# fmazilu/ASR-using-robust-NN

Hardware: AMD Instinct MI355X
Metric: utterances/sec (train, 1 s@16 kHz) (higher is better)
Workload: dtype f32 accumulate, fp16 two-plane split products in the training GEMMs (22-bit operands); 1 GPU; raw 16 kHz waveform -> on-GPU MFCC -> Lipschitz-constrained MLP train step (Adam+NonNeg, simple_norm_constraint rho=0.1), 1xMI355X; global_batch=1024, per_gpu_batch=1024, clip=1 s @ 16 kHz fp32, resident_pool_clips_per_gpu=65536, parallelism=dp1, hip_graph=False

## Files before the change

asr-using-robust-nn_amd/csrc/core.hip:

```cpp
#include "common.h"
#include <map>
#include <mutex>

namespace lipasr {

static thread_local char g_err[512] = "";

void set_error(const char* fmt, ...) {
  va_list ap;
  va_start(ap, fmt);
  vsnprintf(g_err, sizeof(g_err), fmt, ap);
  va_end(ap);
}

int device_cus() {
  static int cached[16] = {};
  int dev = 0; (void)hipGetDevice(&dev);
  int& c = cached[dev & 15];
  if (!c) { hipDeviceProp_t prop; c = hipGetDeviceProperties(&prop, dev) == hipSuccess ? prop.multiProcessorCount : 256; }
  return c;
}

bool ensure_dyn_lds(const void* fn, size_t bytes) {
  if (bytes <= 48 * 1024) return true;
  struct Limit { size_t granted = 0, refused = SIZE_MAX; };
  static std::mutex mu;
  static std::map<std::pair<const void*, int>, Limit> limits;
  int dev = 0; (void)hipGetDevice(&dev);
  std::lock_guard<std::mutex> lock(mu);
  Limit& l = limits[{fn, dev}];
  if (bytes <= l.granted) return true;
  if (bytes >= l.refused) return false;
  if (hipFuncSetAttribute(fn, hipFuncAttributeMaxDynamicSharedMemorySize, (int)bytes) == hipSuccess) { l.granted = bytes; return true; }
  set_error("hipFuncSetAttribute: %zu bytes of dynamic LDS refused: %s", bytes, hipGetErrorString(hipGetLastError()));
  l.refused = bytes;
  return false;
}

void mfcc_plan_free(MfccPlan* p);
void mlp_plan_free(lipasr_mlp* m);
void dolphin_plan_free(DolphinPlan* p);
void psy_plan_free(PsyPlan* p);

}

using namespace lipasr;

extern "C" {

int lipasr_version(void) { return 740; }

const char* lipasr_last_error(void) { return g_err; }

int lipasr_create(int device, lipasr_handle_t* out) {
  LP_CHECK_ARG(out != nullptr, "lipasr_create: out is null");
  int n = 0;
  LP_HIP(hipGetDeviceCount(&n));
  LP_CHECK_ARG(device >= 0 && device < n, "lipasr_create: device %d out of range (have %d)", device, n);
  hipDeviceProp_t prop;
  LP_HIP(hipGetDeviceProperties(&prop, device));
  if (strncmp(prop.gcnArchName, "gfx950", 6) != 0) {
    set_error("lipasr_create: device %d is %s; this library is built for gfx950 only", device, prop.gcnArchName);
    return LIPASR_EUNSUPPORTED;
  }
  DeviceGuard g(device);
  if (!g.ok) { set_error("lipasr_create: hipSetDevice(%d) failed", device); return LIPASR_EHIP; }
  lipasr_ctx* c = new lipasr_ctx();
  c->device = device;
  c->scratch_floats = kScratchFloats;
  if (hipMalloc(&c->scratch, c->scratch_floats * sizeof(float)) != hipSuccess) {
    delete c;
    set_error("lipasr_create: scratch allocation failed");
    return LIPASR_ENOMEM;
  }
  if (hipMemset(c->scratch, 0, c->scratch_floats * sizeof(float)) != hipSuccess) {
    (void)hipFree(c->scratch);
    delete c;
    set_error("lipasr_create: scratch memset failed");
    return LIPASR_EHIP;
  }
  if (hipMalloc(&c->zeros, 256) != hipSuccess || hipMemset(c->zeros, 0, 256) != hipSuccess) {
    (void)hipGetLastError();
    if (c->zeros) (void)hipFree(c->zeros);
    c->zeros = nullptr;
  }
  *out = c;
  return LIPASR_OK;
}

int lipasr_destroy(lipasr_handle_t h) {
  LP_CHECK_ARG(h != nullptr, "lipasr_destroy: null handle");
  DeviceGuard g(h->device);
  (void)hipDeviceSynchronize();
  for (hipGraphExec_t ge : h->graphs)
    if (ge) (void)hipGraphExecDestroy(ge);
  h->graphs.clear();
  for (hipStream_t st : h->streams)
    if (st) (void)hipStreamDestroy(st);
  h->streams.clear();
  std::vector<lipasr_mlp*> mlps;
  mlps.swap(h->mlps);
  for (lipasr_mlp* m : mlps) mlp_plan_free(m);
  std::vector<MfccPlan*> plans;
  plans.swap(h->mfcc_plans);
  for (MfccPlan* p : plans) mfcc_plan_free(p);
  h->mfcc = nullptr;
  std::vector<DolphinPlan*> dolphins;
  dolphins.swap(h->dolphin_plans);
  for (DolphinPlan* p : dolphins) dolphin_plan_free(p);
  std::vector<PsyPlan*> psys;
  psys.swap(h->psy_plans);
  for (PsyPlan* p : psys) psy_plan_free(p);
  for (hipEvent_t e : h->timers) (void)hipEventDestroy(e);
  h->timers.clear();
  if (h->scratch) (void)hipFree(h->scratch);
  if (h->zeros) (void)hipFree(h->zeros);
  delete h;
  return LIPASR_OK;
}

int lipasr_timer_create(lipasr_handle_t h, int* timer_id) {
  LP_CHECK_ARG(h && timer_id, "lipasr_timer_create: null argument");
  DeviceGuard g(h->device);
  hipEvent_t a, b;
  LP_HIP(hipEventCreate(&a));
  LP_HIP(hipEventCreate(&b));
  *timer_id = (int)(h->timers.size() / 2);
  h->timers.push_back(a);
  h->timers.push_back(b);
  return LIPASR_OK;
}

int lipasr_timer_start(lipasr_handle_t h, int id, lipasr_stream_t stream) {
  LP_CHECK_ARG(h && id >= 0 && (size_t)(2 * id + 1) < h->timers.size(), "lipasr_timer_start: bad timer id %d", id);
  LP_HIP(hipEventRecord(h->timers[2 * id], S(stream)));
  return LIPASR_OK;
}

int lipasr_timer_stop(lipasr_handle_t h, int id, lipasr_stream_t stream) {
  LP_CHECK_ARG(h && id >= 0 && (size_t)(2 * id + 1) < h->timers.size(), "lipasr_timer_stop: bad timer id %d", id);
  LP_HIP(hipEventRecord(h->timers[2 * id + 1], S(stream)));
  return LIPASR_OK;
}

int lipasr_timer_elapsed_ms(lipasr_handle_t h, int id, float* ms_host) {
  LP_CHECK_ARG(h && ms_host && id >= 0 && (size_t)(2 * id + 1) < h->timers.size(),
               "lipasr_timer_elapsed_ms: bad argument");
  LP_HIP(hipEventSynchronize(h->timers[2 * id + 1]));
  LP_HIP(hipEventElapsedTime(ms_host, h->timers[2 * id], h->timers[2 * id + 1]));
  return LIPASR_OK;
}

namespace lipasr {
constexpr long long kFlagHardFactor = 4;
__global__ void flag_signal_kernel(int* flag, int value) {
  if (threadIdx.x == 0) __hip_atomic_store(flag, value, __ATOMIC_RELEASE, __HIP_MEMORY_SCOPE_AGENT);
}
__global__ void flag_wait_kernel(const int* flag, int value, int* err, long long soft_ticks) {
  if (threadIdx.x == 0) {
    const long long t0 = wall_clock64();
    bool reported = false;
    while (__hip_atomic_load(flag, __ATOMIC_ACQUIRE, __HIP_MEMORY_SCOPE_AGENT) < value) {
      __builtin_amdgcn_s_sleep(16);
      const long long dt = wall_clock64() - t0;
      if (!reported && dt > soft_ticks) {
        if (__hip_atomic_load(err, __ATOMIC_RELAXED, __HIP_MEMORY_SCOPE_SYSTEM) >= 2) break;
        __hip_atomic_store(err, 1, __ATOMIC_RELAXED, __HIP_MEMORY_SCOPE_SYSTEM);
        reported = true;
      }
      if (dt > kFlagHardFactor * soft_ticks) { __hip_atomic_store(err, 2, __ATOMIC_RELAXED, __HIP_MEMORY_SCOPE_SYSTEM); break; }
    }
  }
}
}

int lipasr_flag_signal(lipasr_handle_t h, int* flag, int value, lipasr_stream_t stream) {
  LP_CHECK_ARG(h && flag, "lipasr_flag_signal: null argument");
  hipLaunchKernelGGL(lipasr::flag_signal_kernel, dim3(1), dim3(64), 0, S(stream), flag, value);
  LP_LAUNCH_CHECK();
  return LIPASR_OK;
}

int lipasr_flag_wait(lipasr_handle_t h, const int* flag, int value, int timeout_ms, int* err, lipasr_stream_t stream) {
  LP_CHECK_ARG(h && flag && err, "lipasr_flag_wait: null argument");
  LP_CHECK_ARG(timeout_ms >= 1 && timeout_ms <= 150000, "lipasr_flag_wait: timeout %d ms outside [1, 150000]", timeout_ms);
  hipLaunchKernelGGL(lipasr::flag_wait_kernel, dim3(1), dim3(64), 0, S(stream), flag, value, err, (long long)timeout_ms * 100000LL);
  LP_LAUNCH_CHECK();
  return LIPASR_OK;
}

int lipasr_graph_begin(lipasr_handle_t h, lipasr_stream_t stream) {
  LP_CHECK_ARG(h != nullptr, "lipasr_graph_begin: null handle");
  LP_HIP(hipStreamBeginCapture(S(stream), hipStreamCaptureModeThreadLocal));
  return LIPASR_OK;
}

int lipasr_graph_end(lipasr_handle_t h, lipasr_stream_t stream, int* graph_id) {
  LP_CHECK_ARG(h && graph_id, "lipasr_graph_end: null argument");
  hipGraph_t graph = nullptr;
  LP_HIP(hipStreamEndCapture(S(stream), &graph));
  hipGraphExec_t exec = nullptr;
  hipError_t e = hipGraphInstantiate(&exec, graph, nullptr, nullptr, 0);
  (void)hipGraphDestroy(graph);
// ... 51 lines not shown
```

asr-using-robust-nn_amd/csrc/mfcc.hip:

```cpp
#include "mfcc_plan.h"
#include <memory>

namespace lipasr {

using namespace tables;

long g_k1_launches[K1_KERNELS] = {};
long g_k1_vjp_launches[K1V_KERNELS] = {};

void mfcc_plan_free(MfccPlan* p) {
  if (!p) return;
  void* ptrs[] = {p->d_hbandh, p->d_groups, p->d_dft, p->d_mel_wlo, p->d_mel_whi, p->d_mel_pstart, p->d_mel_plen, p->d_hband, p->d_lo, p->d_h, p->d_noff, p->d_hann, p->d_tw, p->d_mel_start, p->d_mel_len, p->d_mel_off,
                  p->d_mel_w, p->d_dct, p->d_y, p->d_db, p->d_fmax, p->d_gmel, p->d_part, p->d_gy, p->d_dct_rows, p->d_bin_run, p->d_rt_taps, p->d_rt_t0,
                  p->d_dft_t, p->d_melt_off, p->d_melt_len, p->d_melt_m, p->d_melt_w};
  for (void* q : ptrs)
    if (q) (void)hipFree(q);
  for (hipEvent_t e : p->prof_events) (void)hipEventDestroy(e);
  bdft_tables_free(&p->bd);
  delete p;
}

__global__ __launch_bounds__(256) void add_noise_kernel(float* __restrict__ y, int n, int mode, float p0, float p1,
                                                         uint64_t seed) {
  __shared__ double red[4];
// ... 71 lines not shown
  const bool mfma = p->d_hband && !(p->stage_mask & SM_VALU_RESAMPLER);
  path.resampler = h2 ? MfccPath::RS_H2
                   : p->identity ? MfccPath::RS_COPY
                   : resample_persist_ok(p, wav, fmt) ? MfccPath::RS_PERSIST_F32
                   : mfma ? MfccPath::RS_MFMA
                   : (p->taps == 128 && p->up <= 448) ? MfccPath::RS_REG128 : MfccPath::RS_GENERIC;
  return path;
}
}

using namespace lipasr;

struct lipasr_mfcc : lipasr::MfccPlan {};

namespace lipasr {

static void plan_unregister(MfccPlan* p) {
  if (!p || !p->ctx) return;
  std::vector<MfccPlan*>& v = p->ctx->mfcc_plans;
  for (size_t i = 0; i < v.size(); ++i)
    if (v[i] == p) { v.erase(v.begin() + i); break; }
  if (p->ctx->mfcc == p) p->ctx->mfcc = nullptr;
}

static int plan_build(lipasr_handle_t h, int sr_in, int n_samp, int batch_max, int n_fft, int hop, MfccPlan** out) {
  LP_CHECK_ARG(h != nullptr && out != nullptr, "lipasr_mfcc_plan: null argument");
  const bool dft = !(n_fft == kNFft && hop == kHop);
  if (dft && !(n_fft >= 32 && n_fft <= 32 * kDftMaxTiles * 2 - 2 && hop >= 1 && hop <= n_fft)) {
    set_error("lipasr_mfcc_plan_ex: n_fft=%d hop=%d; supported: 2048/512 (FFT path) or 32 <= n_fft <= %d with "
              "1 <= hop <= n_fft (DFT-contraction path)", n_fft, hop, 32 * kDftMaxTiles * 2 - 2);
    return LIPASR_EUNSUPPORTED;
  }
  LP_CHECK_ARG(sr_in >= 1000 && sr_in <= 384000, "lipasr_mfcc_plan: sr_in=%d outside [1000, 384000]", sr_in);
  LP_CHECK_ARG(n_samp >= 2 && batch_max >= 1, "lipasr_mfcc_plan: n_samp=%d batch_max=%d", n_samp, batch_max);
  DeviceGuard g(h->device);
  std::unique_ptr<MfccPlan, void (*)(MfccPlan*)> guard(new lipasr_mfcc(), mfcc_plan_free);
  MfccPlan* p = guard.get();
  p->ctx = h;
  p->sr_in = sr_in; p->n_samp = n_samp; p->batch_max = batch_max;
  p->identity = (sr_in == kSr);
  resampled_lengths(n_samp, sr_in, kSr, &p->n_valid, &p->n_y);
  if (p->n_y < 2) { set_error("lipasr_mfcc_plan: clip too short after resampling"); return LIPASR_EINVAL; }
  p->n_fft = n_fft; p->hop = hop; p->dft = dft;
  p->rs_target_wgs = h->rs_target_wgs;
  p->n_frames = 1 + p->n_y / hop;
  if (dft && p->n_y <= n_fft / 2) { set_error("lipasr_mfcc_plan_ex: clip shorter than the reflect padding"); return LIPASR_EINVAL; }
  int rc = LIPASR_OK;
  if (!p->identity) {
    Polyphase pp = build_polyphase(sr_in, kSr);
    if (pp.up > 4096 || pp.taps > 2048) {
      set_error("lipasr_mfcc_plan: ratio %d/%d needs %d phases x %d taps; unsupported", pp.up, pp.down, pp.up, pp.taps);
      return LIPASR_EUNSUPPORTED;
    }
    p->up = pp.up; p->down = pp.down; p->taps = pp.taps; p->left = pp.left;
    if ((rc = upload(&p->d_h, pp.h)) != LIPASR_OK || (rc = upload(&p->d_noff, pp.n_off)) != LIPASR_OK) return rc;
    {
      std::vector<float> hb;
      std::vector<int> lo;
      if (build_band_tables(pp, &hb, &lo)) {
        p->n_ptiles = (int)lo.size();
        if ((rc = upload(&p->d_hband, hb)) != LIPASR_OK || (rc = upload(&p->d_lo, lo)) != LIPASR_OK) return rc;
        bool fits = true;
        for (int r = 0; r < (int)lo.size(); ++r) {
          const int first = lo[r] + 1, band0 = first & ~7;
          fits = fits && (first - band0 + kRsBand <= kRhK) && (band0 + kRhK <= kRhRowHalfs);
        }
        if (fits && (rc = upload(&p->d_hbandh, build_band_h2(hb, lo))) != LIPASR_OK) return rc;
      }
    }
    if (!dft && p->d_hband && pp.up == kFuUp && pp.left == 64 && (pp.down % 32) == 0 && pp.down >= 160 && pp.down <= 320 &&
        (kFuQ - 1) * pp.down + lo_max(pp) + 1 + kRsBand <= kFuQ * pp.down + 160) {
      std::vector<int> groups = build_groups(p->n_y, p->n_frames, pp.up);
      if (!groups.empty()) {
        p->n_groups = (int)groups.size() / 4;
        if ((rc = upload(&p->d_groups, groups)) != LIPASR_OK) return rc;
        p->fused = true;
      }
    }
  }
  MelSparse ms = mel_sparse(n_fft);
  if (dft) {
    p->dft_tiles = (1 + n_fft / 2 + 31) / 32;
    p->dft_krows = ((n_fft / 2 + 1 + 2 * kDftGroup - 1) / (2 * kDftGroup)) * (2 * kDftGroup);
    p->dft_rpc = (p->n_y + 2 * (n_fft / 2) + hop - 1) / hop;
    if ((rc = upload(&p->d_dft, dft_table(n_fft, p->dft_krows, p->dft_tiles))) != LIPASR_OK) return rc;
  }
  MelPairs mp = dft ? MelPairs() : mel_pairs();
  if (dft) { mp.wlo.assign(1, 0.f); mp.whi.assign(1, 0.f); mp.start.assign(1, 0); mp.len.assign(1, 0); }
  if (!mp.ok) {
    set_error("lipasr_mfcc_plan: mel filter bank is not a two-filters-per-bin bank");
    return LIPASR_EUNSUPPORTED;
  }
  if ((rc = upload(&p->d_mel_wlo, mp.wlo)) != LIPASR_OK || (rc = upload(&p->d_mel_whi, mp.whi)) != LIPASR_OK ||
      (rc = upload(&p->d_mel_pstart, mp.start)) != LIPASR_OK || (rc = upload(&p->d_mel_plen, mp.len)) != LIPASR_OK ||
      (rc = upload(&p->d_hann, hann_periodic())) != LIPASR_OK || (rc = upload(&p->d_tw, twiddles())) != LIPASR_OK ||
      (rc = upload(&p->d_mel_start, ms.start)) != LIPASR_OK || (rc = upload(&p->d_mel_len, ms.len)) != LIPASR_OK ||
      (rc = upload(&p->d_mel_off, ms.off)) != LIPASR_OK || (rc = upload(&p->d_mel_w, ms.w)) != LIPASR_OK ||
      (rc = upload(&p->d_dct, dct_fragments())) != LIPASR_OK)
    return rc;
  if (!dft && (rc = bdft_tables_build(&p->bd)) != LIPASR_OK) return rc;
  const size_t ny = (size_t)batch_max * p->n_y, ndb = (size_t)batch_max * p->n_frames * 128,
               nfm = (size_t)batch_max * p->n_frames;
  if (hipMalloc(&p->d_y, ny * sizeof(float)) != hipSuccess || hipMalloc(&p->d_db, ndb * sizeof(float)) != hipSuccess ||
      hipMalloc(&p->d_fmax, nfm * sizeof(float)) != hipSuccess) {
    set_error("lipasr_mfcc_plan: intermediate allocation failed");
    return LIPASR_ENOMEM;
  }
  h->mfcc_plans.push_back(p);
  *out = guard.release();
  return LIPASR_OK;
}

static int plan_check(const char* fn, const MfccPlan* p, int batch, int L) {
  LP_CHECK_ARG(p != nullptr, "%s: null plan", fn);
  LP_CHECK_ARG(batch >= 1 && batch <= p->batch_max, "%s: batch %d outside [1, %d]", fn, batch, p->batch_max);
  LP_CHECK_ARG(L >= 1, "%s: utterance_length=%d", fn, L);
  return LIPASR_OK;
}

enum ProfEvent { EV_RESAMPLE_BEGIN, EV_RESAMPLE_END, EV_STFT_BEGIN, EV_STFT_END, EV_DCT_END, kProfEvents };
static hipEvent_t* prof_slot(MfccPlan* p) { return p->prof_n < p->prof_cap ? &p->prof_events[kProfEvents * (size_t)p->prof_n] : nullptr; }

static int plan_resample(MfccPlan* p, const float* wav, int batch, float* y, hipStream_t st) {
  const MfccPath path = pick_mfcc_path(p, wav, 0, false);
  hipEvent_t* ev = prof_slot(p);
  if (ev) LP_HIP(hipEventRecord(ev[EV_RESAMPLE_BEGIN], st));
  int rc = launch_resample(p, path.resampler, wav, 0, nullptr, batch, y, st);
  if (rc != LIPASR_OK) return rc;
  if (ev) {
    LP_HIP(hipEventRecord(ev[EV_RESAMPLE_END], st));
    p->prof_half = true;
  }
  return LIPASR_OK;
}

static int plan_from_22k(MfccPlan* p, const float* y, int batch, int n_y, int L, const double* am, const double* as, float* out,
                         hipStream_t st) {
  LP_CHECK_ARG(n_y == p->n_y, "lipasr_mfcc_from_22k: n_y=%d but the plan was made for %d", n_y, p->n_y);
  LP_CHECK_ARG((am == nullptr) == (as == nullptr), "lipasr_mfcc_from_22k: give both affine arrays or neither");
  const MfccPath path = pick_mfcc_path(p, nullptr, 0, false);
  hipEvent_t* ev = p->prof_half ? prof_slot(p) : nullptr;
  if (ev) LP_HIP(hipEventRecord(ev[EV_STFT_BEGIN], st));
  int rc = launch_from_22k(p, path.stft, y, nullptr, batch, L, am, as, out, st, ev ? ev[EV_STFT_END] : nullptr);
  if (rc != LIPASR_OK) return rc;
  if (ev) {
    LP_HIP(hipEventRecord(ev[EV_DCT_END], st));
    p->prof_half = false;
    p->prof_n++;
  }
  return LIPASR_OK;
}

static int plan_run(MfccPlan* p, const void* wav, int fmt, const int* n_valid, int batch, int L, const double* am, const double* as,
                    float* out, hipStream_t st) {
  LP_CHECK_ARG(wav && out, "lipasr_mfcc: null argument");
  LP_CHECK_ARG(fmt == 0 || fmt == 1, "lipasr_mfcc: sample format %d (0 = float32, 1 = int16 PCM)", fmt);
  LP_CHECK_ARG((am == nullptr) == (as == nullptr), "lipasr_mfcc: give both affine arrays or neither");
  const MfccPath path = pick_mfcc_path(p, wav, fmt, n_valid != nullptr);
  if (path.rc != LIPASR_OK) return path.rc;
  hipEvent_t* ev = p->prof_half ? nullptr : prof_slot(p);
  int rc;
  if (ev) LP_HIP(hipEventRecord(ev[EV_RESAMPLE_BEGIN], st));
  if (path.fused) {
    if (ev) {
      LP_HIP(hipEventRecord(ev[EV_RESAMPLE_END], st));
      LP_HIP(hipEventRecord(ev[EV_STFT_BEGIN], st));
    }
    if ((rc = launch_fused(p, wav, fmt, n_valid, batch, st)) != LIPASR_OK) return rc;
    if (ev) LP_HIP(hipEventRecord(ev[EV_STFT_END], st));
    if ((rc = launch_dct(p, batch, L, am, as, out, n_valid, st)) != LIPASR_OK) return rc;
  } else {
    if ((rc = launch_resample(p, path.resampler, wav, fmt, n_valid, batch, p->d_y, st)) != LIPASR_OK) return rc;
    if (ev) {
      LP_HIP(hipEventRecord(ev[EV_RESAMPLE_END], st));
      LP_HIP(hipEventRecord(ev[EV_STFT_BEGIN], st));
    }
    if ((rc = launch_from_22k(p, path.stft, p->d_y, n_valid, batch, L, am, as, out, st, ev ? ev[EV_STFT_END] : nullptr)) != LIPASR_OK) return rc;
  }
  if (ev) {
    LP_HIP(hipEventRecord(ev[EV_DCT_END], st));
    p->prof_n++;
  }
  return LIPASR_OK;
}

static int vjp_workspaces(const char* fn, MfccPlan* p, size_t n_part) {
  int rc;
  if (!p->d_dct_rows && (rc = upload(&p->d_dct_rows, dct_matrix())) != LIPASR_OK) return rc;
  const size_t ngm = (size_t)p->batch_max * p->n_frames * kNMels, ngy = (size_t)p->batch_max * p->n_y;
  if ((!p->d_gmel && hipMalloc(&p->d_gmel, ngm * sizeof(float)) != hipSuccess) ||
      (!p->d_part && hipMalloc(&p->d_part, n_part * sizeof(float)) != hipSuccess) ||
      (!p->d_gy && hipMalloc(&p->d_gy, ngy * sizeof(float)) != hipSuccess)) {
    (void)hipGetLastError();
    set_error("%s: intermediate allocation failed", fn);
    return LIPASR_ENOMEM;
  }
  return LIPASR_OK;
}

static int vjp_prepare(const char* fn, MfccPlan* p) {
  if (p->vj_ready) return LIPASR_OK;
  DeviceGuard g(p->ctx->device);
  p->vj_groups = (p->n_frames + kVjFrames - 1) / kVjFrames;
  MelPairs mp = mel_pairs();
  std::vector<int> run(kNBins, 0);
  for (int m = 0; m < kNMels; ++m)
    for (int i = 0; i < mp.len[m]; ++i) run[mp.start[m] + i] = m;
  int rc;
  if (!p->d_bin_run && (rc = upload(&p->d_bin_run, run)) != LIPASR_OK) return rc;
  if ((rc = vjp_workspaces(fn, p, (size_t)p->batch_max * p->vj_groups * kVjSeg)) != LIPASR_OK) return rc;
  p->vj_ready = true;
  return LIPASR_OK;
}

static int resample_vjp_prepare(MfccPlan* p) {
  if (p->identity || p->d_rt_taps) return LIPASR_OK;
  DeviceGuard g(p->ctx->device);
  const Polyphase pp = build_polyphase(p->sr_in, kSr);
  const long up = pp.up, down = pp.down;
  auto split = [&](long t, long* q, int* ph) {
    long qq = t / up;
    if (t - qq * up < 0) --qq;
    *q = qq; *ph = (int)(t - qq * up);
  };
  auto pos = [&](long t) { long q; int ph; split(t, &q, &ph); return down * q + pp.n_off[ph]; };
  std::vector<int> t0(pp.down), cnt(pp.down);
  int nt = 0;
  for (int r = 0; r < pp.down; ++r) {
    const long A = (long)r + pp.left - pp.taps, B = (long)r + pp.left - 1;
    long num = A * up, t = num / down;
    if (num - t * down < 0) --t;
    t -= 2;
    while (pos(t) < A) ++t;
    t0[r] = (int)t;
    int c = 0;
    while (pos(t + c) <= B) ++c;
    cnt[r] = c;
    nt = std::max(nt, c);
  }
  std::vector<float> ht((size_t)nt * pp.down, 0.0f);
  for (int r = 0; r < pp.down; ++r)
    for (int i = 0; i < cnt[r]; ++i) {
      long q; int ph;
      split((long)t0[r] + i, &q, &ph);
      const long k = (long)r - (down * q + pp.n_off[ph]) + pp.left - 1;
      if (k >= 0 && k < pp.taps) ht[(size_t)i * pp.down + r] = pp.h[(size_t)ph * pp.taps + k];
    }
  p->rt_nt = nt;
  p->rt_t0min = *std::min_element(t0.begin(), t0.end());
  p->rt_t0max = *std::max_element(t0.begin(), t0.end());
  int rc;
  if ((rc = upload(&p->d_rt_t0, t0)) != LIPASR_OK || (rc = upload(&p->d_rt_taps, ht)) != LIPASR_OK) return rc;
  return LIPASR_OK;
}

static int plan_resample_vjp(MfccPlan* p, const float* gy, int batch, float* gx, hipStream_t st, const int* nv = nullptr) {
  int rc = resample_vjp_prepare(p);
  if (rc != LIPASR_OK) return rc;
  ResampleVjpArgs a;
  a.n_y = p->n_y; a.n_valid = p->n_valid; a.n_samp = p->n_samp; a.up = p->up; a.down = p->down; a.identity = p->identity;
  a.ht = p->d_rt_taps; a.t0 = p->d_rt_t0; a.nt = p->rt_nt; a.t0min = p->rt_t0min; a.t0max = p->rt_t0max;
  a.nv = nv; a.sr_in = p->sr_in;
  return launch_resample_vjp(a, gy, gx, batch, st);
}

static int vjp_short_prepare(const char* fn, MfccPlan* p) {
  if (p->vj_ready) return LIPASR_OK;
  DeviceGuard g(p->ctx->device);
  int n_wgs, seg, rc;
  if ((rc = short_vjp_geometry(p->n_fft, p->hop, p->dft_rpc, p->dft_tiles, p->batch_max, &n_wgs, &seg)) != LIPASR_OK) return rc;
  const int nb = p->dft_tiles * 32, ld = p->dft_tiles * 64;
  const std::vector<float> T = dft_table(p->n_fft, p->dft_krows, p->dft_tiles);
  std::vector<float> TT((size_t)nb * ld, 0.0f);
  for (int b = 0; b < nb; ++b)
    for (int n = 0; n < std::min(nb, p->dft_krows); ++n) {
      const size_t src = (size_t)n * ld + (b >> 5) * 64 + (b & 31), dst = (size_t)b * ld + (n >> 5) * 64 + (n & 31);
      TT[dst] = T[src];
      TT[dst + 32] = T[src + 32];
    }
  const MelSparse ms = mel_sparse(p->n_fft);
  std::vector<int> off(nb, 0), len(nb, 0), mm;
  std::vector<float> ww;
  for (int b = 0; b < nb; ++b) {
    off[b] = (int)mm.size();
    for (int m = 0; m < kNMels; ++m) {
      const int j = b - ms.start[m];
      if (j >= 0 && j < ms.len[m] && ms.w[ms.off[m] + j] != 0.0f) { mm.push_back(m); ww.push_back(ms.w[ms.off[m] + j]); }
    }
    len[b] = (int)mm.size() - off[b];
  }
  if (mm.empty()) { mm.push_back(0); ww.push_back(0.0f); }
  if ((rc = upload(&p->d_melt_off, off)) != LIPASR_OK || (rc = upload(&p->d_melt_len, len)) != LIPASR_OK ||
      (rc = upload(&p->d_melt_m, mm)) != LIPASR_OK || (rc = upload(&p->d_melt_w, ww)) != LIPASR_OK ||
      (rc = vjp_workspaces(fn, p, (size_t)n_wgs * seg)) != LIPASR_OK || (rc = upload(&p->d_dft_t, TT)) != LIPASR_OK)
    return rc;
  p->vj_ready = true;
  return LIPASR_OK;
}

static int ragged_unsupported(const char* fn, const MfccPlan* p) {
  if (!(resample_h2_ok(p, nullptr, 0) && stft2_ok(p))) {
    set_error("%s: per-clip lengths need a 2048/512 plan at 16 kHz or 8 kHz with rows a multiple of 4 samples; this plan is %d Hz, "
              "n_fft %d, rows of %d", fn, p->sr_in, p->n_fft, p->n_samp);
    return LIPASR_EUNSUPPORTED;
  }
  return LIPASR_OK;
}

static int plan_resample_ragged(MfccPlan* p, const void* wav, int fmt, const int* nv, int batch, float* y, hipStream_t st) {
  LP_CHECK_ARG(wav && nv && y, "lipasr_mfcc_plan_resample_ragged: null argument");
  LP_CHECK_ARG(fmt == 0 || fmt == 1, "lipasr_mfcc_plan_resample_ragged: sample format %d (0 = float32, 1 = int16 PCM)", fmt);
  const MfccPath path = pick_mfcc_path(p, wav, fmt, true);
  if (path.rc != LIPASR_OK) return path.rc;
  if (path.fused) {
    set_error("lipasr_mfcc_plan_resample_ragged: this plan runs the fused resample -> STFT kernel for this input (rows of %d samples, "
              "alignment, or plan key 2): it has no resampled signal to return", p->n_samp);
    return LIPASR_EUNSUPPORTED;
  }
  int rc = launch_resample(p, path.resampler, wav, fmt, nv, batch, y, st);
  if (rc != LIPASR_OK) return rc;
  return launch_clear_tail(p, nv, batch, y, st);
}

static int plan_from_22k_ragged(MfccPlan* p, const float* y, const int* nv, int batch, int L, const double* am, const double* as,
                                float* out, hipStream_t st) {
  LP_CHECK_ARG(y && nv && out, "lipasr_mfcc_plan_from_22k_ragged: null argument");
  LP_CHECK_ARG((am == nullptr) == (as == nullptr), "lipasr_mfcc_plan_from_22k_ragged: give both affine arrays or neither");
  const MfccPath path = pick_mfcc_path(p, nullptr, 0, true);
  if (!stft2_ok(p)) {
    set_error("lipasr_mfcc_plan_from_22k_ragged: per-clip lengths need the 2048/512 kernels (n_fft %d, hop %d, stage mask %d)", p->n_fft,
// ... 29 lines not shown
  LP_CHECK_ARG((c.flags & ~(c.entry == VJ_ONE_LENGTH ? 7 : 1)) == 0, "%s: unknown flag bits %d", fn, c.flags);
  if (c.flags & 6) {
    set_error("%s: int16 input and per-clip lengths have no backward pass (float32 rows of one length only)", fn);
    return LIPASR_EUNSUPPORTED;
  }
  if (c.entry == VJ_SHORT && !p->dft) {
    set_error("%s: the short-window backward pass covers the plans made with n_fft, hop other than 2048, 512; this plan is 2048/512 "
              "(lipasr_mfcc_plan_vjp)", fn);
    return LIPASR_EUNSUPPORTED;
  }
  if (c.entry != VJ_SHORT && p->dft) {
    set_error("%s: the backward pass covers the 2048/512 plans; this plan has n_fft %d, hop %d%s", fn, p->n_fft, p->hop,
              c.entry == VJ_ONE_LENGTH ? " (short-window plans: lipasr_mfcc_plan_vjp_short)" : "");
    return LIPASR_EUNSUPPORTED;
  }
  if (c.entry == VJ_ONE_LENGTH && p->n_y <= kNFft) {
    set_error("%s: the backward pass needs clips longer than the reflect padding (n_y %d <= %d)", fn, p->n_y, kNFft);
    return LIPASR_EUNSUPPORTED;
  }
  if (c.entry == VJ_RAGGED) {
    if (c.fmt == 1 && domain == 1) {
      set_error("%s: int16 PCM rows are rows at the plan's input rate (domain 0); the 22 050 Hz signal is float32", fn);
      return LIPASR_EUNSUPPORTED;
    }
    if ((rc = ragged_unsupported(fn, p)) != LIPASR_OK) return rc;
  }
  const MfccPath path = pick_mfcc_path(p, domain == 0 ? c.sig : nullptr, c.fmt, nv != nullptr);
  if (c.entry != VJ_ONE_LENGTH && path.rc != LIPASR_OK) return path.rc;
  if (c.entry == VJ_RAGGED && domain == 0 && path.fused) {
    set_error("%s: this plan runs the fused resample -> STFT kernel for this input (row alignment, or plan key 2), which leaves no "
              "resampled signal behind for the backward pass", fn);
    return LIPASR_EUNSUPPORTED;
  }
  if ((rc = c.entry == VJ_SHORT ? vjp_short_prepare(fn, p) : vjp_prepare(fn, p)) != LIPASR_OK) return rc;
  const MfccPath::Stft stft = p->dft ? MfccPath::ST_DFT : MfccPath::ST_STOCKHAM4;
  const bool reuse_y = (c.flags & 1) && !(c.entry == VJ_ONE_LENGTH && prefers_fused(p));
  const bool reuse_tile = (c.flags & 1) && path.stft == stft && (domain == 1 || reuse_y);
  const float* y = static_cast<const float*>(c.sig);
  if (domain == 0) {
    if (!reuse_y && (rc = launch_resample(p, path.resampler, c.sig, c.fmt, nv, batch, p->d_y, st)) != LIPASR_OK) return rc;
    y = p->d_y;
  }
  if (!reuse_tile && (rc = launch_from_22k(p, stft, y, nv, batch, L, nullptr, nullptr, nullptr, st, nullptr, true)) != LIPASR_OK) return rc;
  MfccVjpArgs a;
  a.y = y; a.n_y = p->n_y; a.n_frames = p->n_frames; a.batch = batch; a.L = L;
  a.db = p->d_db; a.fmax = p->d_fmax; a.g_feat = c.g_feat; a.aff_scale = c.scale; a.dct_rows = p->d_dct_rows;
  a.hann = p->d_hann; a.tw = reinterpret_cast<const float2*>(p->d_tw);
  a.mel_wlo = p->d_mel_wlo; a.mel_whi = p->d_mel_whi; a.bin_run = p->d_bin_run;
  a.gmel = p->d_gmel; a.part = p->d_part; a.n_groups = p->vj_groups;
  a.gy = domain == 0 ? p->d_gy : c.g_sig;
  if (c.entry == VJ_SHORT) {
    if ((rc = launch_mfcc_vjp_db(a, st)) != LIPASR_OK) return rc;
    ShortVjpArgs s;
    s.y = y; s.table = p->d_dft; s.table_t = p->d_dft_t; s.gmel = p->d_gmel;
    s.melt_off = p->d_melt_off; s.melt_len = p->d_melt_len; s.melt_m = p->d_melt_m; s.melt_w = p->d_melt_w;
    s.n_y = p->n_y; s.batch = batch; s.hop = p->hop; s.n_fft = p->n_fft; s.k_rows = p->dft_krows; s.n_tiles = p->dft_tiles;
    s.rpc = p->dft_rpc; s.n_frames = p->n_frames; s.total_rows = batch * p->dft_rpc; s.seg = 0;
    s.part = p->d_part; s.gy = a.gy;
    rc = launch_short_vjp(s, st);
  } else {
    rc = nv ? launch_mfcc_vjp(a, st, nv, p->sr_in, p->n_samp) : launch_mfcc_vjp(a, st);
  }
  if (rc != LIPASR_OK) return rc;
  if (domain == 0) return plan_resample_vjp(p, p->d_gy, batch, c.g_sig, st, nv);
  return LIPASR_OK;
}

static int plan_profile_begin(MfccPlan* p, int max_calls) {
  LP_CHECK_ARG(p != nullptr && max_calls >= 1 && max_calls <= 100000, "lipasr_mfcc_profile_begin: bad argument");
  DeviceGuard g(p->ctx->device);
  while ((int)p->prof_events.size() < kProfEvents * max_calls) {
    hipEvent_t e;
    LP_HIP(hipEventCreate(&e));
    p->prof_events.push_back(e);
  }
  p->prof_cap = max_calls;
  p->prof_n = 0;
  p->prof_half = false;
  return LIPASR_OK;
}

static int plan_profile_end(MfccPlan* p, float* avg_ms3, int* n_calls) {
  LP_CHECK_ARG(p && avg_ms3 && n_calls, "lipasr_mfcc_profile_end: null argument");
  double acc[3] = {0, 0, 0};
  static const int kFrom[3] = {EV_RESAMPLE_BEGIN, EV_STFT_BEGIN, EV_STFT_END}, kTo[3] = {EV_RESAMPLE_END, EV_STFT_END, EV_DCT_END};
  for (int i = 0; i < p->prof_n; ++i) {
    hipEvent_t* ev = &p->prof_events[kProfEvents * (size_t)i];
    LP_HIP(hipEventSynchronize(ev[EV_DCT_END]));
    for (int k = 0; k < 3; ++k) {
      float ms = 0.0f;
      LP_HIP(hipEventElapsedTime(&ms, ev[kFrom[k]], ev[kTo[k]]));
      acc[k] += ms;
    }
  }
  *n_calls = p->prof_n;
  for (int k = 0; k < 3; ++k) avg_ms3[k] = p->prof_n ? (float)(acc[k] / p->prof_n) : 0.0f;
  p->prof_cap = 0;
  p->prof_n = 0;
  p->prof_half = false;
  return LIPASR_OK;
}

static int plan_set(MfccPlan* p, int key, int value) {
  LP_CHECK_ARG(p != nullptr, "lipasr_mfcc_set: null plan");
  LP_CHECK_ARG(key >= 0 && key <= 4, "lipasr_mfcc_set: unknown key %d", key);
  if (key == 3) LP_CHECK_ARG(value >= 4 && value <= 4096 && (value & 3) == 0, "lipasr_mfcc_set: frames per workgroup %d (a multiple of 4)", value);
  if (key == 1) LP_CHECK_ARG(value >= 1 && value <= 4096, "lipasr_mfcc_set: resampler workgroup target %d", value);
  switch (key) {
    case 0: p->stage_mask = value; break;
    case 1: p->rs_target_wgs = value; break;
    case 2: p->prefer_fused = value != 0; break;
    case 3: p->bd_seg = value; break;
    default: p->bd_fuse_dct = value != 0; break;
  }
  return LIPASR_OK;
}

}

extern "C" {

int lipasr_mfcc_create(lipasr_handle_t h, int sr_in, int n_samp_max, int batch_max, int n_fft, int hop, lipasr_mfcc_t* out) {
  LP_CHECK_ARG(out != nullptr, "lipasr_mfcc_create: out is null");
  MfccPlan* p = nullptr;
  int rc = plan_build(h, sr_in, n_samp_max, batch_max, n_fft, hop, &p);
  if (rc != LIPASR_OK) return rc;
  *out = static_cast<lipasr_mfcc*>(p);
  return LIPASR_OK;
}

int lipasr_mfcc_destroy(lipasr_mfcc_t p) {
  LP_CHECK_ARG(p != nullptr, "lipasr_mfcc_destroy: null plan");
  DeviceGuard g(p->ctx->device);
  plan_unregister(p);
  mfcc_plan_free(p);
  return LIPASR_OK;
}

int lipasr_mfcc_plan_dims(lipasr_mfcc_t p, int* n_y, int* n_frames, int* fused) {
  LP_CHECK_ARG(p && n_y && n_frames, "lipasr_mfcc_plan_dims: null argument");
  *n_y = p->n_y;
  *n_frames = p->n_frames;
  if (fused) *fused = p->fused ? 1 : 0;
  return LIPASR_OK;
}

int lipasr_mfcc_extract(lipasr_mfcc_t p, const void* wav, int sample_format, const int* n_valid, int batch, int utterance_length,
                        const double* affine_mean, const double* affine_scale, float* out, lipasr_stream_t stream) {
  int rc = plan_check("lipasr_mfcc_extract", p, batch, utterance_length);
  if (rc != LIPASR_OK) return rc;
  return plan_run(p, wav, sample_format, n_valid, batch, utterance_length, affine_mean, affine_scale, out, S(stream));
}

int lipasr_mfcc_plan_resample(lipasr_mfcc_t p, const float* wav, int batch, float* y, lipasr_stream_t stream) {
  int rc = plan_check("lipasr_mfcc_plan_resample", p, batch, 1);
  if (rc != LIPASR_OK) return rc;
  LP_CHECK_ARG(wav && y, "lipasr_mfcc_plan_resample: null argument");
  return plan_resample(p, wav, batch, y, S(stream));
}

int lipasr_mfcc_plan_from_22k(lipasr_mfcc_t p, const float* y, int batch, int n_y, int utterance_length, const double* affine_mean,
                              const double* affine_scale, float* out, lipasr_stream_t stream) {
  int rc = plan_check("lipasr_mfcc_plan_from_22k", p, batch, utterance_length);
  if (rc != LIPASR_OK) return rc;
  LP_CHECK_ARG(y && out, "lipasr_mfcc_plan_from_22k: null argument");
  return plan_from_22k(p, y, batch, n_y, utterance_length, affine_mean, affine_scale, out, S(stream));
}

int lipasr_mfcc_plan_vjp(lipasr_mfcc_t p, const float* sig, int domain, int batch, int utterance_length, const double* affine_scale,
                         const float* g_feat, float* g_sig, int flags, lipasr_stream_t stream) {
  return plan_vjp(p, {"lipasr_mfcc_plan_vjp", VJ_ONE_LENGTH, sig, 0, nullptr, domain, batch, utterance_length, affine_scale, g_feat, g_sig, flags},
                  S(stream));
}

int lipasr_mfcc_plan_vjp_short(lipasr_mfcc_t p, const float* sig, int domain, int batch, int utterance_length, const double* affine_scale,
                               const float* g_feat, float* g_sig, int flags, lipasr_stream_t stream) {
  return plan_vjp(p, {"lipasr_mfcc_plan_vjp_short", VJ_SHORT, sig, 0, nullptr, domain, batch, utterance_length, affine_scale, g_feat, g_sig, flags},
                  S(stream));
}

int lipasr_mfcc_plan_vjp_ragged(lipasr_mfcc_t p, const void* sig, int sample_format, const int* n_valid, int domain, int batch,
                                int utterance_length, const double* affine_scale, const float* g_feat, float* g_sig, int flags,
                                lipasr_stream_t stream) {
  return plan_vjp(p, {"lipasr_mfcc_plan_vjp_ragged", VJ_RAGGED, sig, sample_format, n_valid, domain, batch, utterance_length, affine_scale,
                      g_feat, g_sig, flags},
                  S(stream));
}

int lipasr_mfcc_plan_resample_ragged(lipasr_mfcc_t p, const void* wav, int sample_format, const int* n_valid, int batch, float* y,
                                     lipasr_stream_t stream) {
  int rc = plan_check("lipasr_mfcc_plan_resample_ragged", p, batch, 1);
  if (rc != LIPASR_OK) return rc;
  return plan_resample_ragged(p, wav, sample_format, n_valid, batch, y, S(stream));
}

int lipasr_mfcc_plan_from_22k_ragged(lipasr_mfcc_t p, const float* y, const int* n_valid, int batch, int utterance_length,
                                     const double* affine_mean, const double* affine_scale, float* out, lipasr_stream_t stream) {
  int rc = plan_check("lipasr_mfcc_plan_from_22k_ragged", p, batch, utterance_length);
  if (rc != LIPASR_OK) return rc;
  return plan_from_22k_ragged(p, y, n_valid, batch, utterance_length, affine_mean, affine_scale, out, S(stream));
}

int lipasr_mfcc_plan_resample_vjp(lipasr_mfcc_t p, const float* g_y, int batch, float* g_wav, lipasr_stream_t stream) {
  int rc = plan_check("lipasr_mfcc_plan_resample_vjp", p, batch, 1);
  if (rc != LIPASR_OK) return rc;
  LP_CHECK_ARG(g_y && g_wav, "lipasr_mfcc_plan_resample_vjp: null argument");
  return plan_resample_vjp(p, g_y, batch, g_wav, S(stream));
}

int lipasr_mfcc_plan_profile_begin(lipasr_mfcc_t p, int max_calls) { return plan_profile_begin(p, max_calls); }
int lipasr_mfcc_plan_profile_end(lipasr_mfcc_t p, float* avg_ms3, int* n_calls) { return plan_profile_end(p, avg_ms3, n_calls); }
int lipasr_mfcc_plan_set(lipasr_mfcc_t p, int key, int value) { return plan_set(p, key, value); }

long lipasr_debug_k1_launches(int kernel) { return (kernel >= 0 && kernel < K1_KERNELS) ? g_k1_launches[kernel] : -1; }

int lipasr_debug_mfcc_stage(lipasr_mfcc_t p, int which, int batch, float* out, lipasr_stream_t stream) {
  LP_CHECK_ARG(p != nullptr && out != nullptr, "lipasr_debug_mfcc_stage: null argument");
  LP_CHECK_ARG(batch >= 1 && batch <= p->batch_max, "lipasr_debug_mfcc_stage: batch %d outside [1, %d]", batch, p->batch_max);
  LP_CHECK_ARG(which >= 0 && which <= 2, "lipasr_debug_mfcc_stage: unknown stage %d (0 dB tile, 1 frame maxima, 2 resampled signal)", which);
  const float* src = which == 0 ? p->d_db : which == 1 ? p->d_fmax : p->d_y;
  const size_t row = which == 0 ? (size_t)p->n_frames * 128 : which == 1 ? (size_t)p->n_frames : (size_t)p->n_y;
  DeviceGuard g(p->ctx->device);
  LP_HIP(hipMemcpyAsync(out, src, (size_t)batch * row * sizeof(float), hipMemcpyDeviceToDevice, S(stream)));
  return LIPASR_OK;
}

long lipasr_debug_k1_vjp_launches(int kernel) { return (kernel >= 0 && kernel < K1V_KERNELS) ? g_k1_vjp_launches[kernel] : -1; }

int lipasr_debug_mfcc_vjp_stage(lipasr_mfcc_t p, int which, int batch, float* out, lipasr_stream_t stream) {
  LP_CHECK_ARG(p != nullptr && out != nullptr, "lipasr_debug_mfcc_vjp_stage: null argument");
  LP_CHECK_ARG(batch >= 1 && batch <= p->batch_max, "lipasr_debug_mfcc_vjp_stage: batch %d outside [1, %d]", batch, p->batch_max);
  LP_CHECK_ARG(which >= 0 && which <= 1, "lipasr_debug_mfcc_vjp_stage: unknown stage %d (0 Gmel, 1 g_y of a domain-0 call)", which);
  LP_CHECK_ARG(p->vj_ready && p->d_gmel && p->d_gy, "lipasr_debug_mfcc_vjp_stage: the plan has run no backward pass yet (no workspaces)");
  const float* src = which == 0 ? p->d_gmel : p->d_gy;
  const size_t row = which == 0 ? (size_t)p->n_frames * 128 : (size_t)p->n_y;
  DeviceGuard g(p->ctx->device);
  LP_HIP(hipMemcpyAsync(out, src, (size_t)batch * row * sizeof(float), hipMemcpyDeviceToDevice, S(stream)));
  return LIPASR_OK;
}

int lipasr_debug_mfcc_stage_put(lipasr_mfcc_t p, int which, int batch, const float* in, lipasr_stream_t stream) {
  LP_CHECK_ARG(p != nullptr && in != nullptr, "lipasr_debug_mfcc_stage_put: null argument");
  LP_CHECK_ARG(batch >= 1 && batch <= p->batch_max, "lipasr_debug_mfcc_stage_put: batch %d outside [1, %d]", batch, p->batch_max);
  LP_CHECK_ARG(which >= 0 && which <= 1, "lipasr_debug_mfcc_stage_put: unknown stage %d (0 dB tile, 1 frame maxima)", which);
  float* dst = which == 0 ? p->d_db : p->d_fmax;
  const size_t row = which == 0 ? (size_t)p->n_frames * 128 : (size_t)p->n_frames;
  DeviceGuard g(p->ctx->device);
  LP_HIP(hipMemcpyAsync(dst, in, (size_t)batch * row * sizeof(float), hipMemcpyDeviceToDevice, S(stream)));
  return LIPASR_OK;
}

int lipasr_mfcc_plan(lipasr_handle_t h, int sr_in, int n_samp, int batch_max) {
  return lipasr_mfcc_plan_ex(h, sr_in, n_samp, batch_max, kNFft, kHop);
}

int lipasr_mfcc_plan_ex(lipasr_handle_t h, int sr_in, int n_samp, int batch_max, int n_fft, int hop) {
  LP_CHECK_ARG(h != nullptr, "lipasr_mfcc_plan: null handle");
  MfccPlan* p = nullptr;
  int rc = plan_build(h, sr_in, n_samp, batch_max, n_fft, hop, &p);
  if (rc != LIPASR_OK) return rc;
  if (h->mfcc) {
    DeviceGuard g(h->device);
    MfccPlan* old = h->mfcc;
    plan_unregister(old);
    mfcc_plan_free(old);
  }
  h->mfcc = p;
  return LIPASR_OK;
}

int lipasr_mfcc_dims(lipasr_handle_t h, int* n_y, int* n_frames) {
  LP_CHECK_ARG(h && n_y && n_frames, "lipasr_mfcc_dims: null argument");
  if (!h->mfcc) { set_error("lipasr_mfcc_dims: call lipasr_mfcc_plan first"); return LIPASR_ESTATE; }
  *n_y = h->mfcc->n_y;
  *n_frames = h->mfcc->n_frames;
  return LIPASR_OK;
}

static int mfcc_check(const char* fn, lipasr_handle_t h, int batch, int L) {
  LP_CHECK_ARG(h != nullptr, "%s: null handle", fn);
  if (!h->mfcc) { set_error("%s: call lipasr_mfcc_plan first", fn); return LIPASR_ESTATE; }
  return plan_check(fn, h->mfcc, batch, L);
}

int lipasr_resample_f32(lipasr_handle_t h, const float* wav, int batch, float* y, lipasr_stream_t stream) {
  int rc = mfcc_check("lipasr_resample_f32", h, batch, 1);
  if (rc != LIPASR_OK) return rc;
  LP_CHECK_ARG(wav && y, "lipasr_resample_f32: null argument");
  return plan_resample(h->mfcc, wav, batch, y, S(stream));
}

int lipasr_mfcc_from_22k(lipasr_handle_t h, const float* y, int batch, int n_y, int utterance_length,
                         const double* affine_mean, const double* affine_scale, float* out, lipasr_stream_t stream) {
  int rc = mfcc_check("lipasr_mfcc_from_22k", h, batch, utterance_length);
  if (rc != LIPASR_OK) return rc;
  LP_CHECK_ARG(y && out, "lipasr_mfcc_from_22k: null argument");
  return plan_from_22k(h->mfcc, y, batch, n_y, utterance_length, affine_mean, affine_scale, out, S(stream));
}

int lipasr_mfcc_f32(lipasr_handle_t h, const float* wav, int batch, int utterance_length, const double* affine_mean,
                    const double* affine_scale, float* out, lipasr_stream_t stream) {
  int rc = mfcc_check("lipasr_mfcc_f32", h, batch, utterance_length);
  if (rc != LIPASR_OK) return rc;
  LP_CHECK_ARG(wav && out, "lipasr_mfcc_f32: null argument");
  LP_CHECK_ARG((affine_mean == nullptr) == (affine_scale == nullptr), "lipasr_mfcc_f32: give both affine arrays or neither");
  return plan_run(h->mfcc, wav, 0, nullptr, batch, utterance_length, affine_mean, affine_scale, out, S(stream));
}

int lipasr_mfcc_i16(lipasr_handle_t h, const int16_t* pcm, const int* n_valid, int batch, int utterance_length,
                    const double* affine_mean, const double* affine_scale, float* out, lipasr_stream_t stream) {
  int rc = mfcc_check("lipasr_mfcc_i16", h, batch, utterance_length);
  if (rc != LIPASR_OK) return rc;
  return plan_run(h->mfcc, pcm, 1, n_valid, batch, utterance_length, affine_mean, affine_scale, out, S(stream));
}

int lipasr_mfcc_profile_begin(lipasr_handle_t h, int max_calls) {
  LP_CHECK_ARG(h != nullptr, "lipasr_mfcc_profile_begin: bad argument");
  if (!h->mfcc) { set_error("lipasr_mfcc_profile_begin: call lipasr_mfcc_plan first"); return LIPASR_ESTATE; }
  return plan_profile_begin(h->mfcc, max_calls);
}

int lipasr_mfcc_profile_end(lipasr_handle_t h, float* avg_ms3, int* n_calls) {
  LP_CHECK_ARG(h && avg_ms3 && n_calls, "lipasr_mfcc_profile_end: null argument");
  if (!h->mfcc) { set_error("lipasr_mfcc_profile_end: call lipasr_mfcc_plan first"); return LIPASR_ESTATE; }
  return plan_profile_end(h->mfcc, avg_ms3, n_calls);
}

int lipasr_add_noise_f32(lipasr_handle_t h, float* y, int batch, int n, int mode, float p0, float p1, uint64_t seed,
                         lipasr_stream_t stream) {
  LP_CHECK_ARG(h && y, "lipasr_add_noise_f32: null argument");
  LP_CHECK_ARG(batch >= 1 && n >= 1, "lipasr_add_noise_f32: bad shape %dx%d", batch, n);
  LP_CHECK_ARG(mode >= 0 && mode <= 2, "lipasr_add_noise_f32: mode %d", mode);
  hipLaunchKernelGGL(add_noise_kernel, dim3(batch), dim3(256), 0, S(stream), y, n, mode, p0, p1, seed);
  LP_LAUNCH_CHECK();
  return LIPASR_OK;
}

int lipasr_debug_set(lipasr_handle_t h, int key, int value) {
  LP_CHECK_ARG(h != nullptr, "lipasr_debug_set: null handle");
  LP_CHECK_ARG(key >= 0 && key <= 2, "lipasr_debug_set: unknown key %d", key);
  if (!h->mfcc) { set_error("lipasr_debug_set: call lipasr_mfcc_plan first"); return LIPASR_ESTATE; }
  int rc = plan_set(h->mfcc, key, value);
  if (rc == LIPASR_OK && key == 1) h->rs_target_wgs = value;
  return rc;
}

int lipasr_debug_table(int which, int sr_in, float* out, int cap) {
  std::vector<float> v;
  switch (which) {
    case 0: v = hann_periodic(); break;
    case 1: v = dct_matrix(); break;
    case 2: v = mel_dense(); break;
    case 3: case 4: case 5: case 6: case 7: {
      LP_CHECK_ARG(sr_in >= 1000 && sr_in != kSr, "lipasr_debug_table: sr_in=%d", sr_in);
      Polyphase pp = build_polyphase(sr_in, kSr);
      if (which == 3) v = pp.h;
      else if (which == 4) v = {(float)pp.up, (float)pp.down, (float)pp.taps, (float)pp.left};
      else if (which == 5) v.assign(pp.n_off.begin(), pp.n_off.end());
      else {
        std::vector<float> hb;
        std::vector<int> lo;
        if (!build_band_tables(pp, &hb, &lo)) { set_error("lipasr_debug_table: no banded form for sr_in=%d", sr_in); return LIPASR_EUNSUPPORTED; }
        if (which == 6) v = hb;
        else v.assign(lo.begin(), lo.end());
      }
      break;
    }
    case 8: {
      MelPairs mp = mel_pairs();
      LP_CHECK_ARG(mp.ok, "lipasr_debug_table: mel bank has no pair form");
      v.assign((size_t)kNMels * kNBins, 0.0f);
      for (int m = 0; m < kNMels; ++m)
        for (int i = 0; i < mp.len[m]; ++i) {
          const int b = mp.start[m] + i;
          v[(size_t)m * kNBins + b] += mp.wlo[b];
          if (m + 1 < kNMels) v[(size_t)(m + 1) * kNBins + b] += mp.whi[b];
        }
// ... 13 lines not shown
```

asr-using-robust-nn_amd/csrc/mfcc_plan.h:

```cpp
#pragma once
#include "common.h"
#include "mfcc_tables.h"
#include "stft.h"

namespace lipasr {

enum StageMask : int {
  SM_SKIP_FFT = 1,
  SM_SKIP_MEL = 2,
  SM_VALU_RESAMPLER = 4,
  SM_MFMA_SKIP_CHAIN = 8,
  SM_NO_H2 = 16,
  SM_MFMA_SKIP_FILL = 16,
  SM_ROUND2_STFT = 64,
  SM_NO_FUSED = 128,
  SM_STOCKHAM = 256,
  SM_FUSED_STOP = 256,
  SM_FUSED_SKIP_RESAMPLE = 512,
  SM_H2_SHIFT = 16, SM_H2_BITS = 7,
  H2_SKIP_MFMA = 1, H2_SKIP_STORE = 2, H2_NO_PREFETCH = 4,
};

constexpr int kRsBand = 152, kRsStride = 481;
constexpr int kRpMaxWaves = 16;
constexpr int kRhK = 160, kRhChunks = kRhK / 16, kRhRowHalfs = 480, kRhRowBytes = 2 * kRhRowHalfs * 2 + 16;
constexpr float kRhTapScale = 64.0f, kRhSigScale = 2048.0f;
constexpr int kFuQ = 16;
constexpr int kFuUp = 441;
constexpr int kDftRows = 64, kDftGroup = 8, kDftMaxTiles = 8;
constexpr int kSvRows = 32;
typedef float rs_f32x16 __attribute__((ext_vector_type(16)));

struct MfccPlan {
  lipasr_ctx* ctx = nullptr;
  int sr_in = 0, n_samp = 0, batch_max = 0;
  int up = 1, down = 1, taps = 0, left = 0;
  int n_valid = 0, n_y = 0, n_frames = 0;
  int n_fft = tables::kNFft, hop = tables::kHop;
  bool dft = false;
  int dft_krows = 0, dft_tiles = 0, dft_rpc = 0;
  float* d_dft = nullptr;
  bool identity = false;
  float* d_h = nullptr;
  int* d_noff = nullptr;
  float* d_hband = nullptr;
  unsigned int* d_hbandh = nullptr;
  int* d_lo = nullptr;
  int n_ptiles = 0;
  int stage_mask = 0;
  int rs_target_wgs = 256;
  int* d_groups = nullptr;
  int n_groups = 0;
  bool fused = false;
  bool prefer_fused = false;
  float* d_hann = nullptr;
  float* d_tw = nullptr;
  int* d_mel_start = nullptr;
  int* d_mel_len = nullptr;
  int* d_mel_off = nullptr;
  float* d_mel_w = nullptr;
  float* d_mel_wlo = nullptr;
  float* d_mel_whi = nullptr;
  int* d_mel_pstart = nullptr;
  int* d_mel_plen = nullptr;
  float* d_dct = nullptr;
  float* d_y = nullptr;
  float* d_db = nullptr;
  float* d_fmax = nullptr;
  std::vector<hipEvent_t> prof_events;
  int prof_cap = 0, prof_n = 0;
  bool prof_half = false;
  BdftTables bd;
  int bd_seg = 44;
  bool bd_fuse_dct = false;
  bool vj_ready = false;
  float* d_gmel = nullptr;
  float* d_part = nullptr;
  float* d_gy = nullptr;
  float* d_dct_rows = nullptr;
  int* d_bin_run = nullptr;
  int vj_groups = 0;
  float* d_rt_taps = nullptr;
  int* d_rt_t0 = nullptr;
  int rt_nt = 0, rt_t0min = 0, rt_t0max = 0;
  float* d_dft_t = nullptr;
  int* d_melt_off = nullptr;
  int* d_melt_len = nullptr;
  int* d_melt_m = nullptr;
  float* d_melt_w = nullptr;
};

struct MfccPath {
  enum Resampler { RS_NONE, RS_H2, RS_PERSIST_F32, RS_MFMA, RS_REG128, RS_GENERIC, RS_COPY };
  enum Stft { ST_BDFT, ST_STOCKHAM4, ST_STOCKHAM2, ST_DFT };
  Resampler resampler = RS_NONE;
  Stft stft = ST_BDFT;
  bool fused = false;
  int rc = LIPASR_OK;
};
MfccPath pick_mfcc_path(const MfccPlan* p, const void* wav, int fmt, bool ragged);

enum K1Kernel { K1_RESAMPLE_H2 = 0, K1_RESAMPLE_PERSIST = 4, K1_RESAMPLE_MFMA, K1_RESAMPLE_REG128, K1_RESAMPLE_GENERIC, K1_COPY_PAD,
                K1_CLEAR_TAIL, K1_STFT_BDFT, K1_STFT_BDFT_DCT, K1_STFT_MEL2, K1_STFT_MEL, K1_DFT_MEL, K1_DCT, K1_FUSED_F32, K1_FUSED_I16,
                K1_KERNELS };
extern long g_k1_launches[K1_KERNELS];
enum K1VjpKernel { K1V_DB = 0, K1V_DB_RAGGED, K1V_STFT, K1V_STFT_RAGGED, K1V_FOLD, K1V_FOLD_RAGGED, K1V_RESAMPLE_Q8, K1V_RESAMPLE_Q1,
                   K1V_RESAMPLE_Q8_RAGGED, K1V_RESAMPLE_Q1_RAGGED, K1V_COPY_CUT, K1V_DFT, K1V_DFT_FOLD, K1V_KERNELS };
extern long g_k1_vjp_launches[K1V_KERNELS];

inline bool rows_vec4(const MfccPlan* p, const void* wav, int fmt) {
  return (reinterpret_cast<uintptr_t>(wav) & (fmt ? 7 : 15)) == 0 && (p->n_samp & 3) == 0;
}

bool build_band_tables(const tables::Polyphase& pp, std::vector<float>* hb_out, std::vector<int>* lo_out);
std::vector<unsigned int> build_band_h2(const std::vector<float>& hb, const std::vector<int>& lo);
int launch_resample(const MfccPlan* p, MfccPath::Resampler kind, const void* wav, int fmt, const int* n_valid, int batch, float* y,
                    hipStream_t st);
int launch_clear_tail(const MfccPlan* p, const int* n_valid, int batch, float* y, hipStream_t st);
std::vector<float> dct_fragments();
void fill_stft_args(const MfccPlan* p, const float* y, StftArgs* a);
int launch_dct(const MfccPlan* p, int batch, int L, const double* am, const double* as, float* out, const int* n_valid, hipStream_t st);
int launch_from_22k(const MfccPlan* p, MfccPath::Stft kind, const float* y, const int* n_valid, int batch, int L, const double* am,
                    const double* as, float* out, hipStream_t st, hipEvent_t mid = nullptr, bool stft_only = false);
int launch_mfcc_vjp_db(const MfccVjpArgs& a, hipStream_t st);
struct ShortVjpArgs {
  const float* y;
  const float* table;
  const float* table_t;
  const float* gmel;
  const int* melt_off;
  const int* melt_len;
  const int* melt_m;
  const float* melt_w;
  int n_y, batch, hop, n_fft, k_rows, n_tiles, rpc, n_frames, total_rows, seg;
  float* part;
  float* gy;
};
int short_vjp_geometry(int n_fft, int hop, int rpc, int n_tiles, int batch, int* n_wgs, int* seg);
int launch_short_vjp(const ShortVjpArgs& a, hipStream_t st);
std::vector<int> build_groups(int n_y, int n_frames, int up);
int launch_fused(const MfccPlan* p, const void* wav, int fmt, const int* n_valid, int batch, hipStream_t st);

}
```

asr-using-robust-nn_amd/csrc/stft_mel.hip:

```cpp
#include "mfcc_plan.h"

namespace lipasr {

using namespace tables;


__global__ __launch_bounds__(256) void stft_mel_kernel(StftArgs a) {
  __shared__ __attribute__((aligned(16))) float2 buf[kFftLds];
  __shared__ float wmax[4];
  __shared__ float2 rsum[2][128];
  const int tid = threadIdx.x;
  int u, fp;
  {
    const int npairs = gridDim.x, L = blockIdx.y * gridDim.x + blockIdx.x;
    const int nb = gridDim.y;
    const int full = (nb / 8) * 8 * npairs;
    if (L < full) {
      const int xcd = L & 7, chunk = L >> 3;
      u = (chunk / npairs) * 8 + xcd;
      fp = chunk % npairs;
    } else {
      u = blockIdx.y;
      fp = blockIdx.x;
    }
// ... 319 lines not shown
  dbe = power_to_db(se);
  dbo = power_to_db(so);
  const int fe = f0 + 2 * pr, fo = fe + 1;
  if (fe < n_frames) a.db[((size_t)u * a.n_frames + fe) * 128 + m] = dbe;
  if (fo < n_frames) a.db[((size_t)u * a.n_frames + fo) * 128 + m] = dbo;
}

__global__ __launch_bounds__(256) __attribute__((amdgpu_waves_per_eu(4, 4))) void stft_mel2_kernel(StftArgs a) {
  __shared__ __attribute__((aligned(16))) float4 buf[kF2Buf];
  __shared__ __attribute__((aligned(16))) float4 rsum[2][128];
  __shared__ float wmax[4][2];
  const int tid = threadIdx.x, lane = tid & 63;
  int u, fq;
  {
    const int nq = gridDim.x, L = blockIdx.y * gridDim.x + blockIdx.x, nb = gridDim.y;
    const int full = (nb / 8) * 8 * nq;
    if (L < full) {
      const int chunk = L >> 3;
      u = (chunk / nq) * 8 + (L & 7);
      fq = chunk % nq;
    } else {
      u = blockIdx.y;
      fq = blockIdx.x;
    }
  }
  const int f0 = 4 * fq;
  const float* yu = a.y + (size_t)u * a.n_y;
  int n_y = a.n_y, n_frames = a.n_frames, n_vy = a.n_y;
  if (a.n_valid) {
    clip_lengths(min(max(a.n_valid[u], 0), a.n_samp_max), a.sr_in, &n_vy, &n_y, &n_frames);
    n_frames = min(n_frames, a.n_frames);
  }
  if (f0 >= n_frames) return;
  float dbe, dbo;
  stft2_quad(a, buf, rsum, yu, u, f0, tid, n_vy, n_y, n_frames, dbe, dbo);
  const float me = wave_max(dbe), mo = wave_max(dbo);
  if (lane == 0) { wmax[tid >> 6][0] = me; wmax[tid >> 6][1] = mo; }
  lds_barrier2();
  if (tid < 4) {
    const int f = f0 + tid, w0 = 2 * (tid >> 1), c = tid & 1;
    if (f < n_frames) a.fmax[(size_t)u * a.n_frames + f] = fmaxf(wmax[w0][c], wmax[w0 + 1][c]);
  }
}
#undef LP_F2_PASS8

struct DftArgs {
  const float* y;
  const float* table;
  int n_y, batch;
  int hop, n_fft, k_rows, n_tiles, rpc, n_frames, total_rows;
  const int* mel_start;
  const int* mel_len;
  const int* mel_off;
  const float* mel_w;
  float* db;
  float* fmax;
};

__global__ __launch_bounds__(64 * kDftMaxTiles) __attribute__((amdgpu_waves_per_eu(4, 4))) void dft_mel_kernel(DftArgs a) {
  extern __shared__ __attribute__((aligned(16))) float dsm[];
  const int tid = threadIdx.x, lane = tid & 63, wave = tid >> 6, nthreads = blockDim.x, n_waves = nthreads >> 6;
  const int row0 = blockIdx.x * kDftRows;
  {
    const int n_a = (kDftRows - 1) * a.hop + a.n_fft + 1;
    const int stride = a.rpc * a.hop, pad = a.n_fft / 2;
    const long g0 = (long)row0 * a.hop;
    for (int i = tid; i < n_a; i += nthreads) {
      const long g = g0 + i;
      const int c = (int)(g / stride);
      const int j = (int)(g - (long)c * stride);
      float v = 0.0f;
      if (c < a.batch && j < a.n_y + 2 * pad) {
        int k = j - pad;
        if (k < 0) k = -k;
        else if (k >= a.n_y) k = 2 * (a.n_y - 1) - k;
        v = a.y[(size_t)c * a.n_y + k];
      }
      dsm[i] = v;
    }
  }
  __syncthreads();
  const int li = lane & 31, kk = lane >> 5;
  const int ld = a.n_tiles * 64;
  rs_f32x16 re0, im0, re1, im1;
#pragma unroll
  for (int q = 0; q < 16; ++q) { re0[q] = 0.f; im0[q] = 0.f; re1[q] = 0.f; im1[q] = 0.f; }
  const float* bp = a.table + (size_t)kk * ld + wave * 64 + li;
  const float* fw0 = dsm + li * a.hop + kk;
  const float* bw0 = dsm + li * a.hop + a.n_fft - kk;
  const float* fw1 = fw0 + 32 * a.hop;
  const float* bw1 = bw0 + 32 * a.hop;
  const int n_groups = a.k_rows / (2 * kDftGroup);
  float br0[kDftGroup], bi0[kDftGroup], br1[kDftGroup], bi1[kDftGroup];
#define LP_DFT_LOAD(BR, BI, G)                                          \
  _Pragma("unroll") for (int u = 0; u < kDftGroup; ++u) {               \
    const float* q_ = bp + (size_t)(2 * ((G) * kDftGroup + u)) * ld;    \
    BR[u] = q_[0];                                                      \
    BI[u] = q_[32];                                                     \
  }
#define LP_DFT_MAC(BR, BI, G)                                           \
  _Pragma("unroll") for (int u = 0; u < kDftGroup; ++u) {               \
    const int s_ = 2 * ((G) * kDftGroup + u);                           \
    const float p0_ = fw0[s_], q0_ = bw0[-s_], p1_ = fw1[s_], q1_ = bw1[-s_]; \
    re0 = __builtin_amdgcn_mfma_f32_32x32x2f32(p0_ + q0_, BR[u], re0, 0, 0, 0); \
    im0 = __builtin_amdgcn_mfma_f32_32x32x2f32(p0_ - q0_, BI[u], im0, 0, 0, 0); \
    re1 = __builtin_amdgcn_mfma_f32_32x32x2f32(p1_ + q1_, BR[u], re1, 0, 0, 0); \
    im1 = __builtin_amdgcn_mfma_f32_32x32x2f32(p1_ - q1_, BI[u], im1, 0, 0, 0); \
  }
  LP_DFT_LOAD(br0, bi0, 0)
  for (int g = 0; g < n_groups; g += 2) {
    if (g + 1 < n_groups) { LP_DFT_LOAD(br1, bi1, g + 1) }
    LP_DFT_MAC(br0, bi0, g)
    if (g + 1 < n_groups) {
      if (g + 2 < n_groups) { LP_DFT_LOAD(br0, bi0, g + 2) }
      LP_DFT_MAC(br1, bi1, g + 1)
    }
  }
#undef LP_DFT_LOAD
#undef LP_DFT_MAC
  __syncthreads();
  const int ldp = a.n_tiles * 32 + 1;
#pragma unroll
  for (int q = 0; q < 16; ++q) {
    const int r = (q & 3) + 8 * (q >> 2) + 4 * kk;
    dsm[r * ldp + wave * 32 + li] = re0[q] * re0[q] + im0[q] * im0[q];
    dsm[(32 + r) * ldp + wave * 32 + li] = re1[q] * re1[q] + im1[q] * im1[q];
  }
  __syncthreads();
  for (int r = wave; r < kDftRows; r += n_waves) {
    const int grow = row0 + r;
    const int clip = grow / a.rpc, frame = grow - clip * a.rpc;
    if (grow >= a.total_rows || frame >= a.n_frames) continue;
    const float* pr = dsm + r * ldp;
    float dbv[2];
#pragma unroll
    for (int hmel = 0; hmel < 2; ++hmel) {
      const int m = lane + 64 * hmel;
      const int st = a.mel_start[m], ln = a.mel_len[m];
      const float* w = a.mel_w + a.mel_off[m];
      float sacc = 0.0f;
      for (int j = 0; j < ln; ++j) sacc = fmaf(w[j], pr[st + j], sacc);
      dbv[hmel] = power_to_db(sacc);
    }
    float* dst = a.db + ((size_t)clip * a.n_frames + frame) * 128;
    dst[lane] = dbv[0];
    dst[lane + 64] = dbv[1];
    const float mx = wave_max(fmaxf(dbv[0], dbv[1]));
    if (lane == 0) a.fmax[(size_t)clip * a.n_frames + frame] = mx;
  }
}


constexpr int kDctFrames = 64;

__global__ __launch_bounds__(128) void dct_kernel(const float* __restrict__ db, const float* __restrict__ frame_max,
                                                   int n_frames, int L, int chunk, const float4* __restrict__ dct_frag,
                                                   const double* __restrict__ aff_mean,
                                                   const double* __restrict__ aff_scale, float* __restrict__ out,
                                                   const int* __restrict__ n_valid, int n_samp_max, int sr_in) {
  extern __shared__ float dbs[];
  __shared__ float red[2];
  const int tid = threadIdx.x, lane = tid & 63, wave = tid >> 6, u = blockIdx.x;
  const int li = lane & 31, h = lane >> 5;
  const int t0 = blockIdx.y * chunk;
  const int tl = min(chunk, L - t0);
  int nf = n_frames;
  if (n_valid) {
    int nvy, ny;
    clip_lengths(min(max(n_valid[u], 0), n_samp_max), sr_in, &nvy, &ny, &nf);
    nf = min(nf, n_frames);
  }
  const int tu = max(0, min(nf - t0, tl));
  const int tp = chunk + 1;
  const float* src = db + ((size_t)u * n_frames + t0) * 128;
  const int n_live = tu * 128;
  float stage[kDctFrames];
#pragma unroll
  for (int j = 0; j < kDctFrames; ++j) {
    const int i = tid + 128 * j;
    stage[j] = (i < n_live) ? src[i] : 0.0f;
  }
  float4 av4[16];
  const float4* ap = dct_frag + (li * 2 + h) * 16;
#pragma unroll
  for (int s4 = 0; s4 < 16; ++s4) av4[s4] = ap[s4];
  float mx = -INFINITY;
  for (int t = tid; t < nf; t += 128) mx = fmaxf(mx, frame_max[(size_t)u * n_frames + t]);
  mx = wave_max(mx);
  if (lane == 0) red[wave] = mx;
  __syncthreads();
  const float thr = fmaxf(red[0], red[1]) - 80.0f;
#pragma unroll
  for (int j = 0; j < kDctFrames; ++j) {
    const int i = tid + 128 * j;
    if (j < chunk) dbs[tid * tp + j] = (i < n_live) ? fmaxf(stage[j], thr) : 0.0f;
  }
  __syncthreads();
  rs_f32x16 acc;
#pragma unroll
  for (int q = 0; q < 16; ++q) acc[q] = 0.0f;
  const float* bp = dbs + h * tp + min(wave * 32 + li, chunk - 1);
#pragma unroll
  for (int s4 = 0; s4 < 16; ++s4) {
    const float a4[4] = {av4[s4].x, av4[s4].y, av4[s4].z, av4[s4].w};
#pragma unroll
    for (int e = 0; e < 4; ++e) acc = __builtin_amdgcn_mfma_f32_32x32x2f32(a4[e], bp[2 * (4 * s4 + e) * tp], acc, 0, 0, 0);
  }
  const int t = wave * 32 + li;
  const int n_out = kNMfcc * L;
  if (t < tl) {
#pragma unroll
    for (int q = 0; q < 16; ++q) {
      const int c = (q & 3) + 8 * (q >> 2) + 4 * h;
      if (c < kNMfcc) {
        float v = (t < tu) ? acc[q] : 0.0f;
        const int oo = c * L + t0 + t;
        if (aff_mean) v = (float)(((double)v - aff_mean[oo]) / aff_scale[oo]);
        out[(size_t)u * n_out + oo] = v;
      }
    }
  }
}

std::vector<float> dct_fragments() {
  const std::vector<float> d = tables::dct_matrix();
  std::vector<float> f((size_t)32 * 2 * 64, 0.0f);
  for (int li = 0; li < kNMfcc; ++li)
    for (int h = 0; h < 2; ++h)
      for (int s = 0; s < 64; ++s) f[((size_t)li * 2 + h) * 64 + s] = d[(size_t)li * 128 + 2 * s + h];
  return f;
}

int launch_dct(const MfccPlan* p, int batch, int L, const double* am, const double* as, float* out, const int* n_valid,
                      hipStream_t st) {
  const int chunk = std::min(kDctFrames, (L + 3) & ~3);
  const size_t lds = (size_t)128 * (chunk + 1) * sizeof(float);
  hipLaunchKernelGGL(dct_kernel, dim3(batch, (L + chunk - 1) / chunk), dim3(128), lds, st, p->d_db, p->d_fmax, p->n_frames, L, chunk,
                     reinterpret_cast<const float4*>(p->d_dct), am, as, out, n_valid, p->n_samp, p->sr_in);
  ++g_k1_launches[K1_DCT];
  LP_LAUNCH_CHECK();
  return LIPASR_OK;
}

void fill_stft_args(const MfccPlan* p, const float* y, StftArgs* a) {
  a->y = y; a->n_y = p->n_y; a->n_frames = p->n_frames; a->hann = p->d_hann;
  a->tw = reinterpret_cast<const float2*>(p->d_tw);
  a->mel_wlo = p->d_mel_wlo; a->mel_whi = p->d_mel_whi; a->mel_start = p->d_mel_pstart; a->mel_len = p->d_mel_plen;
  a->db = p->d_db; a->fmax = p->d_fmax;
  a->stage_mask = p->stage_mask;
  a->n_valid = nullptr; a->sr_in = p->sr_in; a->n_samp_max = p->n_samp;
}

int launch_from_22k(const MfccPlan* p, MfccPath::Stft kind, const float* y, const int* n_valid, int batch, int L, const double* am,
                    const double* as, float* out, hipStream_t st, hipEvent_t mid, bool stft_only) {
  StftArgs a;
  fill_stft_args(p, y, &a);
  a.n_valid = n_valid;
  switch (kind) {
    case MfccPath::ST_DFT: {
      DftArgs d;
      d.y = y; d.n_y = p->n_y; d.batch = batch; d.table = p->d_dft; d.hop = p->hop; d.n_fft = p->n_fft; d.k_rows = p->dft_krows; d.n_tiles = p->dft_tiles;
      d.rpc = p->dft_rpc; d.n_frames = p->n_frames; d.total_rows = batch * p->dft_rpc;
      d.mel_start = p->d_mel_start; d.mel_len = p->d_mel_len; d.mel_off = p->d_mel_off; d.mel_w = p->d_mel_w;
      d.db = p->d_db; d.fmax = p->d_fmax;
      const int n_a = (kDftRows - 1) * p->hop + p->n_fft + 1, n_p = kDftRows * (p->dft_tiles * 32 + 1);
      const size_t dl = (size_t)(n_a > n_p ? n_a : n_p) * sizeof(float);
      LP_DYN_LDS(dft_mel_kernel, dl);
      hipLaunchKernelGGL(dft_mel_kernel, dim3((d.total_rows + kDftRows - 1) / kDftRows), dim3(64 * p->dft_tiles), dl, st, d);
      ++g_k1_launches[K1_DFT_MEL];
      break;
    }
    case MfccPath::ST_BDFT: {
      const bool fuse = !stft_only && p->bd_fuse_dct && bdft_can_fuse_dct(p->n_frames, p->bd_seg, L);
      BdftDct d;
      d.L = L; d.dct_frag = reinterpret_cast<const float4*>(p->d_dct); d.aff_mean = am; d.aff_scale = as; d.out = out;
      const int rc = launch_stft_bdft(a, p->bd, batch, p->bd_seg, fuse ? &d : nullptr, st);
      if (rc != LIPASR_OK) return rc;
      if (fuse) {
        if (mid) LP_HIP(hipEventRecord(mid, st));
        return LIPASR_OK;
      }
      break;
    }
    case MfccPath::ST_STOCKHAM4:
      hipLaunchKernelGGL(stft_mel2_kernel, dim3((p->n_frames + 3) / 4, batch), dim3(256), 0, st, a);
      ++g_k1_launches[K1_STFT_MEL2];
      break;
    case MfccPath::ST_STOCKHAM2:
      hipLaunchKernelGGL(stft_mel_kernel, dim3((p->n_frames + 1) / 2, batch), dim3(256), 0, st, a);
      ++g_k1_launches[K1_STFT_MEL];
      break;
  }
  LP_LAUNCH_CHECK();
  if (mid) LP_HIP(hipEventRecord(mid, st));
  if (stft_only) return LIPASR_OK;
  return launch_dct(p, batch, L, am, as, out, n_valid, st);
}

}
```

asr-using-robust-nn_amd/lipasr/_native.py:

```python
from __future__ import annotations

import ctypes as C
import os

import torch

_HERE = os.path.dirname(os.path.abspath(__file__))
LIB_PATH = os.environ.get("LIPASR_LIBRARY") or os.path.join(_HERE, "liblipasr.so")

if not os.path.exists(LIB_PATH):
    raise ImportError(
        f"{LIB_PATH} not found: build it with `python asr-using-robust-nn_amd/build.py` "
        "(or __graft_entry__.build()).  lipasr has no CPU fallback."
    )

lib = C.CDLL(LIB_PATH)

OK, EINVAL, ENOMEM, EHIP, EUNSUPPORTED, ESTATE = 0, -1, -2, -3, -4, -5
MAX_LAYERS = 16
SEG_W, SEG_B, SEG_GAMMA, SEG_BETA, SEG_MMEAN, SEG_MVAR = range(6)

c_f = C.c_void_p
c_h = C.c_void_p
c_s = C.c_void_p
i32 = C.c_int
f32 = C.c_float
u64 = C.c_uint64
sz = C.c_size_t
PI = C.POINTER(C.c_int)
PV = C.POINTER(C.c_void_p)


class DropoutCfg(C.Structure):
    _fields_ = [("mode", C.c_int), ("seed", C.c_uint64), ("step_dev", C.c_void_p), ("masks", PV)]


PROTOTYPES = {
    "lipasr_version": (i32, []),
    "lipasr_last_error": (C.c_char_p, []),
    "lipasr_create": (i32, [i32, C.POINTER(c_h)]),
    "lipasr_destroy": (i32, [c_h]),
    "lipasr_timer_create": (i32, [c_h, PI]),
    "lipasr_timer_start": (i32, [c_h, i32, c_s]),
    "lipasr_timer_stop": (i32, [c_h, i32, c_s]),
    "lipasr_timer_elapsed_ms": (i32, [c_h, i32, C.POINTER(f32)]),
    "lipasr_graph_begin": (i32, [c_h, c_s]),
    "lipasr_graph_end": (i32, [c_h, c_s, PI]),
    "lipasr_graph_launch": (i32, [c_h, i32, c_s]),
    "lipasr_stream_create_masked": (i32, [c_h, C.POINTER(C.c_uint32), i32, C.POINTER(c_s)]),
    "lipasr_stream_destroy": (i32, [c_h, c_s]),
    "lipasr_graph_destroy": (i32, [c_h, i32]),
    "lipasr_sigma_max": (i32, [c_h, c_f, i32, i32, c_f, i32, i32, i32, c_f, c_s]),
    "lipasr_project_per_layer": (i32, [c_h, PV, PI, PI, i32, f32, c_f, i32, i32, c_f, c_s]),
    "lipasr_project_product": (i32, [c_h, PV, PI, PI, i32, f32, PI, i32, c_f, c_s]),
    "lipasr_product_norm": (i32, [c_h, PV, PI, PI, i32, c_f, c_s]),
    "lipasr_frobenius_project": (i32, [c_h, c_f, sz, f32, c_s]),
    "lipasr_bn_correction": (i32, [c_h, c_f, c_f, i32, c_f, c_s]),
    "lipasr_sv_clip": (i32, [c_h, c_f, i32, i32, f32, c_f, c_f, c_s]),
    "lipasr_sign_step": (i32, [c_h, c_f, c_f, c_f, sz, f32, f32, c_s]),
    "lipasr_lp_step": (i32, [c_h, c_f, c_f, c_f, i32, i32, f32, f32, f32, c_s]),
    "lipasr_lp_ball_init": (i32, [c_h, c_f, c_f, i32, i32, f32, f32, u64, c_f, i32, c_s]),
    "lipasr_scaler_fit": (i32, [c_h, c_f, i32, i32, c_f, c_f, c_s]),
    "lipasr_scaler_apply": (i32, [c_h, c_f, i32, i32, c_f, c_f, c_f, c_s]),
    "lipasr_gemm_f32": (i32, [c_h, i32, i32, i32, i32, i32, c_f, i32, c_f, i32, c_f, i32, c_s]),
    "lipasr_gemm_f16x2": (i32, [c_h, i32, i32, i32, i32, i32, c_f, i32, c_f, i32, c_f, i32, f32, f32, c_s]),
    "lipasr_mlp_create": (i32, [c_h, i32, PI, PI, C.POINTER(f32), PI, i32, C.POINTER(c_h)]),
    "lipasr_mlp_destroy": (i32, [c_h]),
    "lipasr_mlp_sizes": (i32, [c_h, C.POINTER(sz), C.POINTER(sz)]),
    "lipasr_mlp_segment": (i32, [c_h, i32, i32, C.POINTER(sz), C.POINTER(sz)]),
    "lipasr_mlp_train_fwd_bwd": (i32, [c_h, c_f, c_f, c_f, c_f, i32, f32, C.POINTER(DropoutCfg), c_f, c_f, c_f, c_f, c_s]),
    "lipasr_mlp_train_fwd_bwd_head": (i32, [c_h, c_f, c_f, c_f, c_f, i32, f32, C.POINTER(DropoutCfg), c_f, c_f, c_f, c_f, c_s]),
    "lipasr_mlp_train_dw0": (i32, [c_h, c_f, i32, c_f, c_s]),
    "lipasr_mlp_grad_split": (i32, [c_h, C.POINTER(sz)]),
    "lipasr_mlp_train_segments": (i32, [c_h, PI]),
    "lipasr_mlp_train_segment_exchange": (i32, [c_h, i32, i32, C.POINTER(sz)]),
    "lipasr_mlp_part_floats": (i32, [c_h, C.POINTER(sz)]),
    "lipasr_mlp_train_segment": (i32, [c_h, i32, c_f, c_f, c_f, c_f, i32, f32, C.POINTER(DropoutCfg), c_f, c_f, c_f, c_f, c_f, i32, f32, c_s]),
    "lipasr_mlp_adam_nonneg": (i32, [c_h, c_f, c_f, c_f, c_f, c_f, f32, f32, f32, f32, f32, c_s]),
    "lipasr_mlp_project_product": (i32, [c_h, c_f, f32, PI, i32, c_f, c_s]),
    "lipasr_mlp_adam_project_product": (i32, [c_h, c_f, c_f, c_f, c_f, c_f, f32, f32, f32, f32, f32, f32, PI, i32, c_f, c_s]),
    "lipasr_mlp_adam_project_product_signal": (i32, [c_h, c_f, c_f, c_f, c_f, c_f, f32, f32, f32, f32, f32, f32, PI, i32, c_f, C.c_void_p, i32, c_s]),
    "lipasr_mlp_project_per_layer": (i32, [c_h, c_f, f32, c_f, i32, i32, c_f, c_s]),
    "lipasr_mlp_product_norm": (i32, [c_h, c_f, c_f, c_s]),
    "lipasr_mlp_predict": (i32, [c_h, c_f, c_f, c_f, i32, c_f, c_f, c_s]),
    "lipasr_mlp_input_grad": (i32, [c_h, c_f, c_f, c_f, c_f, i32, c_f, c_s]),
    "lipasr_mlp_set_compute": (i32, [c_h, i32]),
    "lipasr_mlp_set_gemm_tiles": (i32, [c_h, i32]),
    "lipasr_mlp_set_fuse_bn": (i32, [c_h, i32]),
    "lipasr_mlp_set_cu_budget": (i32, [c_h, i32]),
    "lipasr_mlp_exchange_errors": (i32, [c_h, C.POINTER(C.c_int)]),
    "lipasr_mlp_output_vjp": (i32, [c_h, c_f, c_f, c_f, c_f, i32, i32, c_f, c_f, c_s]),
    "lipasr_mlp_jacobian": (i32, [c_h, c_f, c_f, c_f, i32, i32, c_f, c_f, C.c_long, C.c_long, c_s]),
    "lipasr_jacobian_sigma": (i32, [c_h, c_f, i32, i32, i32, C.c_long, C.c_long, c_f, c_f, c_f, c_s]),
    "lipasr_deepfool_step": (i32, [c_h, c_f, C.c_long, C.c_long, c_f, c_f, c_f, i32, i32, i32, f32, f32, f32, f32, c_f, c_f, c_f, c_f, c_s]),
    "lipasr_smooth_expand": (i32, [c_h, c_f, c_f, i32, i32, i32, C.c_uint32, C.c_uint32, f32, u64, f32, f32, c_f, c_s]),
    "lipasr_smooth_vote": (i32, [c_h, c_f, i32, i32, i32, c_f, c_s]),
    "lipasr_smooth_noise_host": (i32, [u64, C.c_uint32, C.c_uint32, i32, C.POINTER(f32)]),
    "lipasr_genetic_breed": (i32, [c_h, c_f, c_f, c_f, c_f, i32, i32, i32, C.c_uint32, C.c_uint32, u64, C.c_uint32, f32, f32, f32, f32, c_f, c_s]),
    "lipasr_genetic_breed_host": (i32, [c_f, c_f, c_f, c_f, i32, i32, i32, C.c_uint32, C.c_uint32, u64, C.c_uint32, f32, f32, f32, f32, c_f]),
    "lipasr_genetic_select": (i32, [c_h, c_f, c_f, i32, i32, i32, i32, f32, C.c_uint32, C.c_uint32, u64, c_f, c_f, c_f, c_f, c_s]),
    "lipasr_apgd_loss": (i32, [c_h, c_f, c_f, i32, i32, i32, i32, c_f, c_f, c_f, c_s]),
    "lipasr_apgd_step": (i32, [c_h, c_f, c_f, c_f, c_f, c_f, c_f, c_f, c_f, c_f, c_f, c_f, c_f, c_f, c_f, c_f, c_f, c_f, c_f, i32, i32, f32, f32,
                               f32, f32, f32, f32, f32, i32, i32, c_s]),
    "lipasr_debug_apgd_path": (i32, [i32, i32]),
    "lipasr_square_init": (i32, [c_h, c_f, c_f, i32, i32, i32, C.c_uint32, C.c_uint32, u64, f32, f32, f32, c_f, c_f, c_f, c_s]),
    "lipasr_square_step": (i32, [c_h, c_f, c_f, c_f, c_f, i32, i32, i32, i32, i32, i32, C.c_uint32, i32, C.c_uint32, C.c_uint32, C.c_uint32,
                                 i32, u64, f32, f32, f32, c_f, c_f, c_f, c_f, c_f, c_s]),
    "lipasr_square_init_host": (i32, [c_f, c_f, i32, i32, i32, C.c_uint32, C.c_uint32, u64, f32, f32, f32, c_f, c_f, c_f]),
    "lipasr_square_step_host": (i32, [c_f, c_f, c_f, c_f, i32, i32, i32, i32, i32, i32, C.c_uint32, i32, C.c_uint32, C.c_uint32, C.c_uint32,
                                      i32, u64, f32, f32, f32, c_f, c_f, c_f, c_f, c_f]),
    "lipasr_hsj_expand": (i32, [c_h, c_f, c_f, c_f, i32, i32, i32, C.c_uint32, C.c_uint32, C.c_uint32, u64, f32, f32, f32, c_f, c_s]),
    "lipasr_hsj_accumulate": (i32, [c_h, c_f, c_f, c_f, c_f, c_f, i32, i32, i32, i32, i32, c_f, c_f, c_s]),
    "lipasr_hsj_direction": (i32, [c_h, c_f, c_f, c_f, i32, i32, f32, c_f, c_s]),
    "lipasr_hsj_search": (i32, [c_h, c_f, c_f, c_f, c_f, c_f, c_f, c_f, c_f, i32, i32, i32, i32, i32, i32, C.c_uint32, C.c_uint32, u64, f32,
                                f32, i32, f32, f32, c_f, c_f, c_f, c_f, c_f, c_f, c_s]),
    "lipasr_hsj_expand_host": (i32, [c_f, c_f, c_f, i32, i32, i32, C.c_uint32, C.c_uint32, C.c_uint32, u64, f32, f32, f32, c_f]),
    "lipasr_hsj_accumulate_host": (i32, [c_f, c_f, c_f, c_f, c_f, i32, i32, i32, i32, i32, c_f, c_f]),
    "lipasr_hsj_direction_host": (i32, [c_f, c_f, c_f, i32, i32, f32, c_f]),
    "lipasr_hsj_search_host": (i32, [c_f, c_f, c_f, c_f, c_f, c_f, c_f, c_f, i32, i32, i32, i32, i32, i32, C.c_uint32, C.c_uint32, u64, f32, f32,
                                     i32, f32, f32, c_f, c_f, c_f, c_f, c_f, c_f]),
    "lipasr_debug_hsj_path": (i32, [i32, i32]),
    "lipasr_room_apply": (i32, [c_f, c_f, c_f, i32, i32, i32, i32, c_f, c_s]),
    "lipasr_room_vjp": (i32, [c_f, c_f, c_f, i32, i32, i32, i32, f32, c_f, c_s]),
    "lipasr_room_apply_host": (i32, [c_f, c_f, c_f, i32, i32, i32, i32, c_f]),
    "lipasr_room_vjp_host": (i32, [c_f, c_f, c_f, i32, i32, i32, i32, f32, c_f]),
    "lipasr_universal_shifts": (i32, [c_h, i32, i32, C.c_uint32, C.c_uint32, u64, c_f, c_s]),
    "lipasr_universal_apply": (i32, [c_h, c_f, c_f, c_f, c_f, i32, i32, i32, f32, f32, c_f, c_s]),
    "lipasr_universal_reduce": (i32, [c_h, c_f, c_f, c_f, i32, i32, i32, c_f, c_s]),
    "lipasr_universal_step": (i32, [c_h, c_f, c_f, i32, i32, f32, f32, f32, c_s]),
    "lipasr_universal_shifts_host": (i32, [i32, i32, C.c_uint32, C.c_uint32, u64, c_f]),
    "lipasr_universal_apply_host": (i32, [c_f, c_f, c_f, c_f, i32, i32, i32, f32, f32, c_f]),
    "lipasr_universal_reduce_host": (i32, [c_f, c_f, c_f, i32, i32, i32, c_f]),
    "lipasr_universal_step_host": (i32, [c_f, c_f, i32, i32, f32, f32, f32]),
    "lipasr_mlp_bounds_workspace": (i32, [c_h, i32, C.POINTER(sz)]),
    "lipasr_mlp_bounds": (i32, [c_h, c_f, c_f, c_f, c_f, f32, f32, f32, c_f, i32, c_f, sz, c_f, c_f, c_f, c_f, c_f, c_s]),
    "lipasr_mlp_bounds_workspace_host": (i32, [i32, PI, i32, C.POINTER(sz)]),
    "lipasr_mlp_bounds_host": (i32, [i32, PI, PI, c_f, c_f, c_f, c_f, f32, f32, f32, c_f, i32, c_f, sz, c_f, c_f, c_f, c_f, c_f]),
    "lipasr_debug_bounds_launches": (C.c_long, [i32]),
    "lipasr_warp_table_host": (i32, [c_f, c_f]),
    "lipasr_warp_apply": (i32, [c_f, c_f, c_f, c_f, i32, i32, i32, c_f, c_s]),
    "lipasr_warp_param_vjp": (i32, [c_f, c_f, c_f, c_f, c_f, i32, i32, i32, c_f, c_s]),
    "lipasr_warp_apply_host": (i32, [c_f, c_f, c_f, c_f, i32, i32, i32, c_f]),
    "lipasr_warp_param_vjp_host": (i32, [c_f, c_f, c_f, c_f, c_f, i32, i32, i32, c_f]),
    "lipasr_debug_warp_launches": (C.c_long, [i32]),
    "lipasr_defence_apply": (i32, [c_f, c_f, PI, PI, PV, i32, i32, i32, c_f, c_s]),
    "lipasr_defence_vjp": (i32, [c_f, c_f, c_f, PI, PI, PV, i32, i32, i32, c_f, c_s]),
    "lipasr_defence_apply_host": (i32, [c_f, c_f, PI, PI, PV, i32, i32, i32, c_f]),
    "lipasr_defence_vjp_host": (i32, [c_f, c_f, c_f, PI, PI, PV, i32, i32, i32, c_f]),
    "lipasr_debug_defence_launches": (C.c_long, [i32]),
    "lipasr_mlp_attack_step": (i32, [c_h, c_f, c_f, c_f, c_f, c_f, i32, f32, f32, c_s]),
    "lipasr_mlp_attack_step_lp": (i32, [c_h, c_f, c_f, c_f, c_f, c_f, i32, f32, f32, f32, c_s]),
    "lipasr_mlp_own_labels": (i32, [c_h, c_f, c_f, c_f, i32, c_f, c_s]),
    "lipasr_mfcc_plan": (i32, [c_h, i32, i32, i32]),
    "lipasr_mfcc_plan_ex": (i32, [c_h, i32, i32, i32, i32, i32]),
    "lipasr_mfcc_dims": (i32, [c_h, PI, PI]),
    "lipasr_mfcc_f32": (i32, [c_h, c_f, i32, i32, c_f, c_f, c_f, c_s]),
    "lipasr_resample_f32": (i32, [c_h, c_f, i32, c_f, c_s]),
    "lipasr_mfcc_from_22k": (i32, [c_h, c_f, i32, i32, i32, c_f, c_f, c_f, c_s]),
    "lipasr_mfcc_i16": (i32, [c_h, c_f, c_f, i32, i32, c_f, c_f, c_f, c_s]),
    "lipasr_mfcc_create": (i32, [c_h, i32, i32, i32, i32, i32, C.POINTER(c_h)]),
    "lipasr_mfcc_destroy": (i32, [c_h]),
    "lipasr_mfcc_plan_dims": (i32, [c_h, PI, PI, PI]),
    "lipasr_mfcc_extract": (i32, [c_h, c_f, i32, c_f, i32, i32, c_f, c_f, c_f, c_s]),
    "lipasr_mfcc_plan_resample": (i32, [c_h, c_f, i32, c_f, c_s]),
    "lipasr_mfcc_plan_from_22k": (i32, [c_h, c_f, i32, i32, i32, c_f, c_f, c_f, c_s]),
    "lipasr_mfcc_plan_vjp": (i32, [c_h, c_f, i32, i32, i32, c_f, c_f, c_f, i32, c_s]),
    "lipasr_mfcc_plan_resample_vjp": (i32, [c_h, c_f, i32, c_f, c_s]),
    "lipasr_mfcc_plan_vjp_short": (i32, [c_h, c_f, i32, i32, i32, c_f, c_f, c_f, i32, c_s]),
    "lipasr_mfcc_plan_vjp_ragged": (i32, [c_h, c_f, i32, c_f, i32, i32, i32, c_f, c_f, c_f, i32, c_s]),
    "lipasr_mfcc_plan_resample_ragged": (i32, [c_h, c_f, i32, c_f, i32, c_f, c_s]),
    "lipasr_mfcc_plan_from_22k_ragged": (i32, [c_h, c_f, c_f, i32, i32, c_f, c_f, c_f, c_s]),
    "lipasr_mfcc_plan_profile_begin": (i32, [c_h, i32]),
    "lipasr_mfcc_plan_profile_end": (i32, [c_h, C.POINTER(f32), PI]),
    "lipasr_mfcc_plan_set": (i32, [c_h, i32, i32]),
    "lipasr_mfcc_profile_begin": (i32, [c_h, i32]),
    "lipasr_mfcc_profile_end": (i32, [c_h, C.POINTER(f32), PI]),
    "lipasr_dolphin_create": (i32, [c_h, i32, i32, i32, C.c_double, C.c_double, C.POINTER(c_h)]),
    "lipasr_dolphin_destroy": (i32, [c_h]),
    "lipasr_dolphin_bandpass": (i32, [c_h, c_f, c_f, i32, c_f, c_s]),
    "lipasr_dolphin_generate": (i32, [c_h, c_f, c_f, i32, c_f, c_f, c_s]),
    "lipasr_dolphin_record": (i32, [c_h, c_f, c_f, i32, f32, f32, c_f, c_s]),
    "lipasr_dolphin_generate_recorded": (i32, [c_h, c_f, c_f, i32, f32, f32, c_f, c_s]),
    "lipasr_dolphin_table": (i32, [i32, i32, C.POINTER(C.c_double), i32]),
    "lipasr_psy_create": (i32, [c_h, i32, i32, i32, i32, C.POINTER(c_h)]),
    "lipasr_psy_destroy": (i32, [c_h]),
    "lipasr_psy_psd": (i32, [c_h, c_f, i32, i32, c_f, c_f, c_s]),
    "lipasr_psy_threshold": (i32, [c_h, c_f, i32, i32, c_f, c_f, c_s]),
    "lipasr_psy_prepare": (i32, [c_h, c_f, i32, i32, c_f, c_f, c_s]),
    "lipasr_psy_loss_grad": (i32, [c_h, c_f, i32, i32, c_f, c_f, c_f, c_f, c_s]),
    "lipasr_psy_step": (i32, [c_h, c_f, c_f, c_f, c_f, c_f, c_f, c_f, i32, i32, f32, i32, f32, f32, c_s]),
    "lipasr_psy_table": (i32, [i32, i32, C.POINTER(C.c_double), i32]),
    "lipasr_add_noise_f32": (i32, [c_h, c_f, i32, i32, i32, f32, f32, u64, c_s]),
    "lipasr_debug_set": (i32, [c_h, i32, i32]),
    "lipasr_debug_gemm_mode": (i32, [i32]),
    "lipasr_debug_launch_count": (C.c_long, [i32]),
    "lipasr_debug_gemm_launches": (C.c_long, [i32, i32, i32, i32, i32, i32]),
    "lipasr_debug_group_launches": (C.c_long, [i32, i32, i32]),
    "lipasr_debug_k3_launches": (C.c_long, [i32]),
    "lipasr_debug_k1_launches": (C.c_long, [i32]),
    "lipasr_debug_mfcc_stage": (i32, [c_h, i32, i32, c_f, c_s]),
    "lipasr_debug_k1_vjp_launches": (C.c_long, [i32]),
    "lipasr_debug_mfcc_vjp_stage": (i32, [c_h, i32, i32, c_f, c_s]),
    "lipasr_debug_mfcc_stage_put": (i32, [c_h, i32, i32, c_f, c_s]),
    "lipasr_debug_k2_launches": (C.c_long, [i32]),
    "lipasr_debug_mlp_stage": (i32, [c_h, i32, i32, i32, c_f, c_s]),
    "lipasr_debug_gemm": (i32, [c_h, i32, i32, i32, i32, i32, i32, c_f, i32, c_f, i32, c_f, i32, f32, f32, c_s]),
    "lipasr_flag_signal": (i32, [c_h, C.c_void_p, i32, c_s]),
    "lipasr_flag_wait": (i32, [c_h, C.c_void_p, i32, i32, C.c_void_p, c_s]),
    "lipasr_debug_chain_head": (i32, [i32]),
    "lipasr_debug_table": (i32, [i32, i32, C.POINTER(f32), i32]),
}

SINCE = {"lipasr_mlp_adam_project_product_signal": 560, "lipasr_dolphin_create": 570, "lipasr_dolphin_destroy": 570,
         "lipasr_dolphin_bandpass": 570, "lipasr_dolphin_generate": 570, "lipasr_dolphin_record": 570,
         "lipasr_dolphin_generate_recorded": 570, "lipasr_dolphin_table": 570, "lipasr_mlp_jacobian": 580,
         "lipasr_jacobian_sigma": 580, "lipasr_psy_create": 590, "lipasr_psy_destroy": 590, "lipasr_psy_psd": 590,
         "lipasr_psy_threshold": 590, "lipasr_psy_prepare": 590, "lipasr_psy_loss_grad": 590, "lipasr_psy_step": 590,
         "lipasr_psy_table": 590, "lipasr_deepfool_step": 600, "lipasr_smooth_expand": 610,
         "lipasr_smooth_vote": 610, "lipasr_smooth_noise_host": 610, "lipasr_genetic_breed": 620,
         "lipasr_genetic_breed_host": 620, "lipasr_genetic_select": 620, "lipasr_debug_k3_launches": 630,
         "lipasr_debug_k1_launches": 640, "lipasr_debug_mfcc_stage": 640, "lipasr_apgd_loss": 650, "lipasr_apgd_step": 650,
         "lipasr_debug_apgd_path": 650, "lipasr_square_init": 660, "lipasr_square_step": 660, "lipasr_square_init_host": 660,
         "lipasr_square_step_host": 660, "lipasr_hsj_expand": 670, "lipasr_hsj_accumulate": 670, "lipasr_hsj_direction": 670,
         "lipasr_hsj_search": 670, "lipasr_hsj_expand_host": 670, "lipasr_hsj_accumulate_host": 670, "lipasr_hsj_direction_host": 670,
         "lipasr_hsj_search_host": 670, "lipasr_debug_hsj_path": 670, "lipasr_room_apply": 680, "lipasr_room_vjp": 680,
         "lipasr_room_apply_host": 680, "lipasr_room_vjp_host": 680, "lipasr_debug_k1_vjp_launches": 690,
         "lipasr_debug_mfcc_vjp_stage": 690, "lipasr_debug_mfcc_stage_put": 690, "lipasr_universal_shifts": 700,
         "lipasr_universal_apply": 700, "lipasr_universal_reduce": 700, "lipasr_universal_step": 700,
         "lipasr_universal_shifts_host": 700, "lipasr_universal_apply_host": 700, "lipasr_universal_reduce_host": 700,
         "lipasr_universal_step_host": 700, "lipasr_mlp_bounds_workspace": 710, "lipasr_mlp_bounds": 710,
         "lipasr_mlp_bounds_workspace_host": 710, "lipasr_mlp_bounds_host": 710, "lipasr_debug_bounds_launches": 710, "lipasr_warp_table_host": 720,
         "lipasr_warp_apply": 720, "lipasr_warp_param_vjp": 720, "lipasr_warp_apply_host": 720, "lipasr_warp_param_vjp_host": 720,
         "lipasr_debug_warp_launches": 720, "lipasr_debug_k2_launches": 730, "lipasr_debug_mlp_stage": 730, "lipasr_defence_apply": 740,
         "lipasr_defence_vjp": 740, "lipasr_defence_apply_host": 740, "lipasr_defence_vjp_host": 740, "lipasr_debug_defence_launches": 740}
lib.lipasr_version.restype = i32
_VERSION = lib.lipasr_version()


def has(name) -> bool:
    return _VERSION >= SINCE.get(name, 0)


for _name, (_res, _args) in PROTOTYPES.items():
    if not has(_name):
        continue
    _fn = getattr(lib, _name)
    _fn.restype = _res
    _fn.argtypes = _args


if os.environ.get("LIPASR_CHAIN_HEAD"):
    lib.lipasr_debug_chain_head(int(os.environ["LIPASR_CHAIN_HEAD"]))
if os.environ.get("LIPASR_GEMM_MODE"):
    lib.lipasr_debug_gemm_mode(int(os.environ["LIPASR_GEMM_MODE"]))


def last_error() -> str:
    return (lib.lipasr_last_error() or b"").decode("utf-8", "replace")


class LipasrError(RuntimeError):
    def __init__(self, code: int, msg: str):
        super().__init__(f"liblipasr error {code}: {msg}")
        self.code = code


def check(rc: int) -> int:
    if rc >= 0:
        return rc
    msg = last_error()
    if rc == EINVAL:
        raise ValueError(f"liblipasr: {msg}")
    raise LipasrError(rc, msg)


def int_array(values):
    arr = (C.c_int * max(1, len(values)))(*[int(v) for v in values])
    return arr


def float_array(values):
    return (C.c_float * max(1, len(values)))(*[float(v) for v in values])


def ptr_array(ptrs):
    return (C.c_void_p * max(1, len(ptrs)))(*[C.c_void_p(int(p) if p else None) for p in ptrs])


def ptr(t):
    if t is None:
        return None
    return C.c_void_p(t.data_ptr())


def stream_ptr():
    import torch

    return C.c_void_p(torch.cuda.current_stream().cuda_stream)


_handles = {}
_owners = []


def register_owner(obj):
    import weakref

    _owners.append(weakref.ref(obj))
    if len(_owners) > 256:
        _owners[:] = [r for r in _owners if r() is not None]


_capture_depth = 0
_deferred = []


def capture_enter():
    global _capture_depth
    _capture_depth += 1


def capture_exit():
    global _capture_depth
    _capture_depth = max(0, _capture_depth - 1)
    if _capture_depth == 0:
        pending, _deferred[:] = list(_deferred), []
        for fn, args in pending:
            fn(*args)


def destroy_or_defer(fn, *args):
    if _capture_depth > 0:
        _deferred.append((fn, args))
    else:
        fn(*args)


class Handle:

    def __init__(self, device: int):
        self.device = device
        h = c_h()
        check(lib.lipasr_create(device, C.byref(h)))
        self.h = h

    @property
    def alive(self):
        return bool(self.h)

    def close(self):
        if self.h:
            for ref in reversed(list(_owners)):
                obj = ref()
                if obj is not None and (getattr(obj, "h", None) is self or getattr(obj, "_h", None) is self):
                    try:
                        obj.close()
                    except Exception:
                        pass
            lib.lipasr_destroy(self.h)
            self.h = None


def get_handle(device=None) -> Handle:
    import torch

    if not torch.cuda.is_available():
        raise RuntimeError("lipasr needs an MI355X (gfx950) GPU: torch.cuda.is_available() is False and there is no CPU path")
    if device is None:
        device = torch.cuda.current_device()
    h = _handles.get(device)
    if h is None or not h.alive:
        h = _handles[device] = Handle(device)
    return h


def shutdown():
    global _capture_depth
    _capture_depth = 0
    pending, _deferred[:] = list(_deferred), []
    for fn, args in pending:
        try:
            fn(*args)
        except Exception:
            pass
    owners, _owners[:] = list(_owners), []
    for ref in reversed(owners):
        obj = ref()
# ... 470 lines not shown
```

asr-using-robust-nn_amd/lipasr/extract_features_construct_dataset.py:

```python
from __future__ import annotations

import ctypes as C
import wave

import numpy as np
import torch

from . import _native as N
from . import estimators as E
from .keras import Model

STANDARD_UTTERANCE_LENGTH = 44
N_MFCC = 20


class MfccExtractor:

    def __init__(self, sr_in=16000, n_samp=16000, batch_max=512, device=None, n_fft=2048, hop=512):
        self.device = torch.device("cuda", torch.cuda.current_device()) if device is None else torch.device(device)
        self.h = N.get_handle(self.device.index)
        self.sr_in, self.n_samp, self.batch_max = int(sr_in), int(n_samp), int(batch_max)
        self.n_fft, self.hop = int(n_fft), int(hop)
        self.short_window = (self.n_fft, self.hop) != (2048, 512)
        plan = N.c_h()
        N.check(N.lib.lipasr_mfcc_create(self.h.h, self.sr_in, self.n_samp, self.batch_max, int(n_fft), int(hop), C.byref(plan)))
        self._plan = plan
        N.register_owner(self)
        ny, nf, fu = C.c_int(), C.c_int(), C.c_int()
        N.check(N.lib.lipasr_mfcc_plan_dims(plan, C.byref(ny), C.byref(nf), C.byref(fu)))
        self.n_y, self.n_frames, self.fused = ny.value, nf.value, bool(fu.value)

    def close(self):
        plan, self._plan = getattr(self, "_plan", None), None
        if plan and self.h.alive:
            N.destroy_or_defer(N.lib.lipasr_mfcc_destroy, plan)

    def __del__(self):
        try:
            self.close()
        except Exception:
            pass

    def set(self, key, value):
        N.check(N.lib.lipasr_mfcc_plan_set(self._plan, int(key), int(value)))

    def profile_begin(self, max_calls):
        N.check(N.lib.lipasr_mfcc_plan_profile_begin(self._plan, int(max_calls)))

    def profile_end(self):
        ms3, n = (C.c_float * 3)(), C.c_int()
        N.check(N.lib.lipasr_mfcc_plan_profile_end(self._plan, ms3, C.byref(n)))
        return {"resample": ms3[0], "stft_mel": ms3[1], "dct": ms3[2]}, n.value

    def __call__(self, waves, utterance_length=STANDARD_UTTERANCE_LENGTH, mean=None, scale=None, out=None, n_valid=None):
        if self._plan is None:
            raise RuntimeError("MfccExtractor used after close()")
        b = waves.shape[0]
        if waves.shape[1] != self.n_samp or not waves.is_contiguous():
            raise ValueError(f"waves must be contiguous [B, {self.n_samp}], got {tuple(waves.shape)}")
        if waves.dtype == torch.int16:
            fmt = 1
        elif waves.dtype == torch.float32:
            fmt = 0
        else:
            raise ValueError(f"waves must be float32 or int16, got {waves.dtype}")
        if n_valid is not None and (n_valid.dtype != torch.int32 or n_valid.shape[0] != b):
            raise ValueError("n_valid must be an int32 device tensor [B]")
        if out is None:
            out = torch.empty(b, N_MFCC * utterance_length, device=self.device)
        N.check(N.lib.lipasr_mfcc_extract(self._plan, N.ptr(waves), fmt, N.ptr(n_valid), b, utterance_length, N.ptr(mean), N.ptr(scale),
                                          N.ptr(out), N.stream_ptr()))
        return out

    def _lengths(self, n_valid, b):
        if not torch.is_tensor(n_valid) or n_valid.dtype != torch.int32 or tuple(n_valid.shape) != (b,) or not n_valid.is_cuda \
                or not n_valid.is_contiguous():
            raise ValueError(f"n_valid must be a contiguous int32 device tensor [{b}]")
        return n_valid

    def resample(self, waves, out=None, n_valid=None):
        y = torch.empty(waves.shape[0], self.n_y, device=self.device) if out is None else out
        if n_valid is None:
            N.check(N.lib.lipasr_mfcc_plan_resample(self._plan, N.ptr(waves), waves.shape[0], N.ptr(y), N.stream_ptr()))
            return y
        b = waves.shape[0]
        if waves.dim() != 2 or waves.shape[1] != self.n_samp or not waves.is_contiguous() or waves.dtype not in (torch.float32, torch.int16):
            raise ValueError(f"waves must be contiguous float32 or int16 [B, {self.n_samp}], got {waves.dtype} {tuple(waves.shape)}")
        if tuple(y.shape) != (b, self.n_y) or y.dtype != torch.float32 or not y.is_contiguous():
            raise ValueError(f"out must be contiguous float32 [{b}, {self.n_y}]")
        N.check(N.lib.lipasr_mfcc_plan_resample_ragged(self._plan, N.ptr(waves), 1 if waves.dtype == torch.int16 else 0,
                                                       N.ptr(self._lengths(n_valid, b)), b, N.ptr(y), N.stream_ptr()))
        return y

    def from_22k(self, y, utterance_length=STANDARD_UTTERANCE_LENGTH, mean=None, scale=None, out=None, n_valid=None):
        if out is None:
            out = torch.empty(y.shape[0], N_MFCC * utterance_length, device=self.device)
        if n_valid is None:
            N.check(N.lib.lipasr_mfcc_plan_from_22k(self._plan, N.ptr(y), y.shape[0], y.shape[1], utterance_length, N.ptr(mean), N.ptr(scale),
                                                    N.ptr(out), N.stream_ptr()))
            return out
        b = y.shape[0]
        if y.dim() != 2 or y.shape[1] != self.n_y or y.dtype != torch.float32 or not y.is_contiguous():
            raise ValueError(f"y must be contiguous float32 [B, {self.n_y}], got {y.dtype} {tuple(y.shape)}")
        if tuple(out.shape) != (b, N_MFCC * utterance_length) or out.dtype != torch.float32 or not out.is_contiguous():
            raise ValueError(f"out must be contiguous float32 [{b}, {N_MFCC * utterance_length}]")
        N.check(N.lib.lipasr_mfcc_plan_from_22k_ragged(self._plan, N.ptr(y), N.ptr(self._lengths(n_valid, b)), b, int(utterance_length),
                                                       N.ptr(mean), N.ptr(scale), N.ptr(out), N.stream_ptr()))
        return out

    def _vjp_args(self, sig, g_feat, utterance_length, scale, domain, out, dtypes):
        if self._plan is None:
            raise RuntimeError("MfccExtractor used after close()")
        if domain not in ("input", "22k"):
            raise ValueError(f"domain={domain!r}: 'input' or '22k'")
        dom = 0 if domain == "input" else 1
        n = self.n_samp if dom == 0 else self.n_y
        b = sig.shape[0]
        if sig.dim() != 2 or sig.shape[1] != n or not sig.is_contiguous():
            raise ValueError(f"sig must be contiguous [B, {n}] for domain {domain!r}, got {tuple(sig.shape)}")
        if sig.dtype not in dtypes:
            raise ValueError(f"sig must be {' or '.join(str(d).split('.')[-1] for d in dtypes)}, got {sig.dtype}")
        if tuple(g_feat.shape) != (b, N_MFCC * utterance_length) or g_feat.dtype != torch.float32 or not g_feat.is_contiguous():
            raise ValueError(f"g_feat must be contiguous float32 [{b}, {N_MFCC * utterance_length}]")
        if scale is not None and (scale.dtype != torch.float64 or scale.numel() != N_MFCC * utterance_length):
            raise ValueError("scale must be a float64 device tensor [20 * utterance_length]")
        if out is None:
            out = torch.empty(b, n, device=self.device)
        elif tuple(out.shape) != (b, n) or out.dtype != torch.float32 or not out.is_contiguous():
            raise ValueError(f"out must be contiguous float32 [{b}, {n}]")
        return dom, b, out

    def vjp(self, sig, g_feat, utterance_length=STANDARD_UTTERANCE_LENGTH, scale=None, domain="input", reuse_forward=False, out=None,
            n_valid=None):
        dom, b, out = self._vjp_args(sig, g_feat, utterance_length, scale, domain, out, (torch.float32, torch.int16))
        flags = (1 if reuse_forward else 0) | (2 if sig.dtype == torch.int16 else 0) | (4 if n_valid is not None else 0)
        N.check(N.lib.lipasr_mfcc_plan_vjp(self._plan, N.ptr(sig), dom, b, int(utterance_length), N.ptr(scale), N.ptr(g_feat), N.ptr(out),
                                           flags, N.stream_ptr()))
        return out

    def vjp_short(self, sig, g_feat, utterance_length, scale=None, domain="22k", reuse_forward=False, out=None):
        dom, b, out = self._vjp_args(sig, g_feat, utterance_length, scale, domain, out, (torch.float32,))
        N.check(N.lib.lipasr_mfcc_plan_vjp_short(self._plan, N.ptr(sig), dom, b, int(utterance_length), N.ptr(scale), N.ptr(g_feat),
                                                 N.ptr(out), 1 if reuse_forward else 0, N.stream_ptr()))
        return out

    def vjp_ragged(self, sig, g_feat, n_valid, utterance_length=STANDARD_UTTERANCE_LENGTH, scale=None, domain="input", reuse_forward=False,
                   out=None):
        dom, b, out = self._vjp_args(sig, g_feat, utterance_length, scale, domain, out, (torch.float32, torch.int16))
        N.check(N.lib.lipasr_mfcc_plan_vjp_ragged(self._plan, N.ptr(sig), 1 if sig.dtype == torch.int16 else 0, N.ptr(self._lengths(n_valid, b)),
                                                  dom, b, int(utterance_length), N.ptr(scale), N.ptr(g_feat), N.ptr(out),
                                                  1 if reuse_forward else 0, N.stream_ptr()))
        return out

    def resample_vjp(self, g_y, out=None):
        if g_y.dim() != 2 or g_y.shape[1] != self.n_y or g_y.dtype != torch.float32 or not g_y.is_contiguous():
            raise ValueError(f"g_y must be contiguous float32 [B, {self.n_y}]")
        if out is None:
            out = torch.empty(g_y.shape[0], self.n_samp, device=self.device)
        N.check(N.lib.lipasr_mfcc_plan_resample_vjp(self._plan, N.ptr(g_y), g_y.shape[0], N.ptr(out), N.stream_ptr()))
        return out


_extractors = {}


def _extractor(sr_in, n_samp, batch_max):
    key = (sr_in, n_samp, torch.cuda.current_device())
    ex = _extractors.get(key)
    if ex is None or ex.batch_max < batch_max or ex._plan is None or not ex.h.alive:
        if len(_extractors) >= 8:
            _extractors.pop(next(iter(_extractors))).close()
        ex = MfccExtractor(sr_in, n_samp, batch_max)
        _extractors[key] = ex
    return ex


def mfcc(waveforms, sr_in=16000, utterance_length=STANDARD_UTTERANCE_LENGTH, n_valid=None):
    dev = torch.device("cuda", torch.cuda.current_device())
    if torch.is_tensor(waveforms):
        w = waveforms
    else:
        a = np.asarray(waveforms)
        w = torch.as_tensor(a if a.dtype == np.int16 else a.astype(np.float32))
    if w.dtype != torch.int16:
        w = w.to(dtype=torch.float32)
    w = w.to(device=dev).contiguous()
    nv = None
    if n_valid is not None:
        nv = torch.as_tensor(np.asarray(n_valid, dtype=np.int32)).to(dev) if not torch.is_tensor(n_valid) else n_valid.to(device=dev, dtype=torch.int32)
    return _extractor(int(sr_in), w.shape[1], w.shape[0])(w, utterance_length, n_valid=nv)


def read_wav(file_path, pcm16=False):
    with wave.open(str(file_path), "rb") as f:
        sr, nch, width, n = f.getframerate(), f.getnchannels(), f.getsampwidth(), f.getnframes()
        raw = f.readframes(n)
    if pcm16 and width == 2 and nch == 1:
        return np.frombuffer(raw, dtype="<i2").copy(), sr
    if width == 2:
        x = np.frombuffer(raw, dtype="<i2").astype(np.float32) / 32768.0
    elif width == 1:
        x = (np.frombuffer(raw, dtype=np.uint8).astype(np.float32) - 128.0) / 128.0
    elif width == 4:
        x = np.frombuffer(raw, dtype="<i4").astype(np.float32) / 2147483648.0
    else:
        raise ValueError(f"unsupported sample width {width} in {file_path}")
    if nch > 1:
        x = x.reshape(-1, nch).mean(axis=1).astype(np.float32)
    return x, sr


def extract_features(file_path, utterance_length):
    x, sr = read_wav(file_path)
    out = mfcc(x[None, :], sr, utterance_length)
    return out.view(N_MFCC, utterance_length).cpu().numpy()


def compute_mfcc_all_files(filenames, chunk=512):
    feats = np.zeros((len(filenames), N_MFCC * STANDARD_UTTERANCE_LENGTH))
    by_sr = {}
    for i, fn in enumerate(filenames):
        x, sr = read_wav(fn, pcm16=True)
# ... 230 lines not shown
```

asr-using-robust-nn_amd/lipasr/pipeline.py:

```python
from __future__ import annotations

import ctypes as C

import torch

from . import _native as N
from .attacks import _norm_value
from .extract_features_construct_dataset import MfccExtractor
from .parallel import DataParallel


class TrainPipeline:
    def __init__(self, model, batch, sr_in=16000, n_samp=16000, utterance_length=44, rho=0.1, constraint="product",
                 affine=None, pgd=None, dp=None, use_graph="auto", per_layer_iters=4, extractor=None, mfcc_cus="auto",
                 sync_inputs=True, overlap_buckets=False, sync_bn=False, train_cus="auto"):
        self.sync_inputs = bool(sync_inputs)
        if pgd:
            self._pgd_norm = _norm_value(pgd.get("norm", float("inf")))
            rinit = int(pgd.get("num_random_init", 0))
            if rinit not in (0, 1):
                raise ValueError(f"pgd num_random_init={rinit}: 0 or 1 (more restarts inside training are not supported)")
            self._pgd_rinit = rinit == 1
            self._pgd_seed = (0xBA11000000000000 + int(model._seed)) & 0xFFFFFFFFFFFFFFFF
        self._train_cus = train_cus
        self.overlap_buckets = bool(overlap_buckets)
        self.model, self.batch, self.L = model, int(batch), int(utterance_length)
        self.dev = model._device
        self.h = N.get_handle(self.dev.index)
        self.ex = MfccExtractor(sr_in, n_samp, self.batch, self.dev) if extractor is None else extractor
        self._custom_ex = extractor is not None
        self.rho, self.constraint, self.pgd = float(rho), constraint, pgd
        self.dp = dp if dp is not None else DataParallel()
        model._replica_rank = self.dp.rank
        self._late = model.late_floats
        self.sync_bn = bool(sync_bn) and self.dp.world > 1
        self.use_graph = (bool(pgd) or self.sync_bn) if use_graph == "auto" else bool(use_graph)
        self.per_layer_iters = per_layer_iters
        self.mean, self.scale = affine if affine is not None else (None, None)
        nf = 20 * self.L
        if model._widths[0] != nf:
            raise ValueError(f"model input width {model._widths[0]} != {nf}")
        self._nbuf = 2
        self._feats2 = [torch.zeros(self.batch, nf, device=self.dev) for _ in range(self._nbuf)]
        self._labels2 = [torch.zeros(self.batch, model._n_classes, device=self.dev) for _ in range(self._nbuf)]
        self.feats, self.labels = self._feats2[0], self._labels2[0]
        self.x_adv = torch.zeros(self.batch, nf, device=self.dev) if pgd else None
        nl = len(model._blocks)
        self.norms = torch.zeros(nl + 1, device=self.dev)
        self.sigmas = torch.zeros(nl, device=self.dev)
        self.v_state = torch.zeros(sum(model._widths[1:]), device=self.dev)
        self._order = N.int_array(list(range(nl)))
        self._warm = False
        self._masked_stream = self._masked_train_stream = None
        self._gemm_tiles_set = False
        self.stream = torch.cuda.Stream(device=self.dev)
        self.mfcc_stream = self._make_mfcc_stream(mfcc_cus)
        import os as _os

        self._wide_stream = torch.cuda.Stream(device=self.dev) if (self._masked_stream is not None and not self._custom_ex
                                                                  and _os.environ.get("LIPASR_WIDE_WHEN_IDLE", "1") == "1") else None
        self._ev_last_mfcc = None
        self._last_xs = None
        self._last_train_ev = None
        self._n_cu = torch.cuda.get_device_properties(self.dev).multi_processor_count
        self._flags = None
        self._flag_err = None
        want_flags = _os.environ.get("LIPASR_GPU_FLAGS", "auto")
        if want_flags == "auto":
            want_flags = "1" if (self.dp.world == 1 and not self.sync_bn) else "0"
        if want_flags == "1" and self._masked_train_stream is not None:
            self._flags = torch.zeros(2 * self._nbuf, dtype=torch.int32, device=self.dev)
            self._flag_err = torch.zeros(1, dtype=torch.int32).pin_memory()
            self._flag_timeout_ms = int(_os.environ.get("LIPASR_FLAG_TIMEOUT_MS", "30000"))
        self._adam_signal = (self._flags is not None and self.dp.world == 1 and not self.sync_bn and not self.use_graph
                             and self.constraint == "product" and N.has("lipasr_mlp_adam_project_product_signal")
                             and _os.environ.get("LIPASR_ADAM_SIGNAL", "1") == "1")
        self._ev_feat = [torch.cuda.Event() for _ in range(self._nbuf)]
        self._ev_free = [None] * self._nbuf
        self._i = 0
        self._graphs = {}
        self._closed = False
        self._prof = None
        N.register_owner(self)

    def _make_mfcc_stream(self, mfcc_cus):
        import os

        n_cu = torch.cuda.get_device_properties(self.dev).multi_processor_count
        if mfcc_cus == "auto":
            env = os.environ.get("LIPASR_MFCC_CUS")
            if env is not None:
                mfcc_cus = int(env)
            elif self._custom_ex:
                mfcc_cus = (n_cu * 7) // 8
            else:
                rest = self._train_cus == "rest" or (self._train_cus == "auto" and not self.pgd
                                                     and os.environ.get("LIPASR_TRAIN_CUS", "rest") == "rest")
                if rest:
                    mfcc_cus = n_cu // 4 if self.batch <= 768 else ((n_cu * 3) // 8 if self.batch <= 1536 else n_cu // 2)
                    if getattr(self.model, "_compute_dtype", "float32") == "float16x2" and 768 < self.batch <= 1536:
                        mfcc_cus = n_cu // 2
                else:
                    mfcc_cus = n_cu // 2
        if not mfcc_cus or mfcc_cus >= n_cu:
            if self.pgd:
                self._own_queue_train_stream(n_cu)
            return torch.cuda.Stream(device=self.dev)
        n_groups = max(1, n_cu // 8)
        k = max(4, min((int(mfcc_cus) // 32) * 4, n_groups))
        words = (n_cu + 31) // 32
        mask = (C.c_uint32 * words)()
        for g in range(k):
            for b in range(8 * g, 8 * g + 8):
                mask[b // 32] |= 1 << (b % 32)
        self.mfcc_cus = 8 * k
        st = N.c_s()
        rc = N.lib.lipasr_stream_create_masked(self.h.h, mask, words, C.byref(st))
        if rc != N.OK:
            import warnings

            warnings.warn(f"lipasr: CU-masked stream unavailable ({N.last_error()}); the MFCC stream shares every CU")
            if self.pgd:
                self._own_queue_train_stream(n_cu)
            return torch.cuda.Stream(device=self.dev)
        self._masked_stream = st
        if hasattr(self.ex, "set"):
            self.ex.set(1, self.mfcc_cus)
        want = self._train_cus if self._train_cus != "auto" else os.environ.get("LIPASR_TRAIN_CUS", "all" if (self._custom_ex or self.pgd) else "rest")
        if want == "rest" and k < n_groups:
            mask2 = (C.c_uint32 * words)()
            for g in range(k, n_groups):
                for b in range(8 * g, 8 * g + 8):
                    mask2[b // 32] |= 1 << (b % 32)
            st2 = N.c_s()
            if N.lib.lipasr_stream_create_masked(self.h.h, mask2, words, C.byref(st2)) == N.OK:
                self._masked_train_stream = st2
                self.stream = torch.cuda.ExternalStream(st2.value, device=self.dev)
                self.train_cus = 8 * (n_groups - k)
                N.check(N.lib.lipasr_mlp_set_gemm_tiles(self.model._plan, int(os.environ.get("LIPASR_GEMM_TILES", "128"))))
                N.check(N.lib.lipasr_mlp_set_cu_budget(self.model._plan, self.train_cus))
                self._gemm_tiles_set = True
        else:
            self._own_queue_train_stream(n_cu)
        return torch.cuda.ExternalStream(st.value, device=self.dev)

    def _own_queue_train_stream(self, n_cu):
        import os

        if os.environ.get("LIPASR_TRAIN_OWN_QUEUE", "1") != "1":
            return
        words = (n_cu + 31) // 32
        mask2 = (C.c_uint32 * words)()
        for b in range(n_cu):
            mask2[b // 32] |= 1 << (b % 32)
        st2 = N.c_s()
        if N.lib.lipasr_stream_create_masked(self.h.h, mask2, words, C.byref(st2)) == N.OK:
            self._masked_train_stream = st2
            self.stream = torch.cuda.ExternalStream(st2.value, device=self.dev)

    def _check_flags(self):
        fe = self._flag_err
        if fe is None:
            return
        code = int(fe[0])
        if code:
            fe[0] = 0
            self._failed = True
            what = ("is overdue (it is still waiting: nothing ran out of order)" if code == 1
                    else "gave up: what its stream did afterwards was not ordered against the other stream")
            raise RuntimeError(f"TrainPipeline: a device-side wait between the extraction and the classifier stream {what} "
                               f"after {self._flag_timeout_ms} ms without the other stream's signal; LIPASR_GPU_FLAGS=0 uses events")

    def _pgd_loop(self, bsz, x, y):
        m = self.model
        eps, eps_step = float(self.pgd["eps"]), float(self.pgd.get("eps_step", 0.1))
        xa = self.x_adv[:bsz]
        if self._pgd_rinit:
            N.check(N.lib.lipasr_lp_ball_init(self.h.h, N.ptr(xa), N.ptr(x), bsz, xa.shape[1], self._pgd_norm, eps, self._pgd_seed,
                                              N.ptr(m._step), self.dp.rank, N.stream_ptr()))
        else:
            xa.copy_(x)
        for _ in range(int(self.pgd.get("max_iter", 20))):
            if self._pgd_norm == float("inf"):
                N.check(N.lib.lipasr_mlp_attack_step(m._plan, N.ptr(m._params), N.ptr(m._bnstate), N.ptr(xa), N.ptr(x), N.ptr(y), bsz,
                                                     eps_step, eps, N.stream_ptr()))
            else:
                N.check(N.lib.lipasr_mlp_attack_step_lp(m._plan, N.ptr(m._params), N.ptr(m._bnstate), N.ptr(xa), N.ptr(x), N.ptr(y), bsz,
                                                        self._pgd_norm, eps_step, eps, N.stream_ptr()))
        return xa

    def _attack_and_train(self, bsz, b, global_batch, defer_dw0=False):
        m = self.model
        x = self._feats2[b][:bsz]
        y = self._labels2[b][:bsz]
        if self.pgd:
            x = self._pgd_loop(bsz, x, y)
        m.train_fwd_bwd(x, y, inv_batch=1.0 / float(global_batch), defer_dw0=defer_dw0)

    def _attack_only(self, bsz, b):
        x = self._feats2[b][:bsz]
        if not self.pgd:
            return x
        return self._pgd_loop(bsz, x, self._labels2[b][:bsz])

    def _syncbn_step(self, bsz, b, gb):
        m = self.model
        n_seg = m.syncbn_segments()
        y = self._labels2[b][:bsz]
        xin = (self.x_adv if self.pgd else self._feats2[b])[:bsz]
        if not self.use_graph:
            self._attack_only(bsz, b)
            for seg in range(n_seg):
                n = m.syncbn_segment(seg, xin, y, gb, self.dp.world)
                if n:
                    self.dp.allreduce_grads(m._part[:n])
            self.dp.allreduce_grads(m._grads)
            self._update()
            return
        key = (bsz, b, gb, "syncbn")
        g = self._graphs.get(key)
        if g is None:
            counts = []

            def first():
                self._attack_only(bsz, b)
                counts.append(m.syncbn_segment(0, xin, y, gb, self.dp.world))

            ids = [self._capture(first)]
            for seg in range(1, n_seg):
                ids.append(self._capture(lambda s=seg: counts.append(m.syncbn_segment(s, xin, y, gb, self.dp.world))))
            ids.append(self._capture(self._update))
            self._sync_counts = getattr(self, "_sync_counts", {})
            self._sync_counts[key] = counts
            g = tuple(ids)
            self._graphs[key] = g
        counts = self._sync_counts[key]
        for seg in range(n_seg):
            N.check(N.lib.lipasr_graph_launch(self.h.h, g[seg], N.stream_ptr()))
            if counts[seg]:
                self.dp.allreduce_grads(m._part[:counts[seg]])
        self.dp.allreduce_grads(m._grads)
        N.check(N.lib.lipasr_graph_launch(self.h.h, g[n_seg], N.stream_ptr()))

    def _dw0(self, bsz, b):
        self.model.train_dw0((self.x_adv if self.pgd else self._feats2[b])[:bsz])

    def _reduce_and_update_eager(self, bsz, b):
        m = self.model
        late = self._late
        ha = self.dp.allreduce_async(m._grads[late:])
        self._dw0(bsz, b)
        hb = self.dp.allreduce_async(m._grads[:late])
        ha.wait()
        hb.wait()
        self._update()

    def _update(self, free_flag=None):
        m = self.model
        if self.constraint == "product":
            m.apply_adam_project_product(self.rho, self._order, self.norms, flag=free_flag, value=self._i)
            return
        m.apply_adam()
        if self.constraint == "per_layer":
            N.check(N.lib.lipasr_mlp_project_per_layer(m._plan, N.ptr(m._params), self.rho, N.ptr(self.v_state), 1, self.per_layer_iters,
                                                       N.ptr(self.sigmas), N.stream_ptr()))

    def _capture(self, fn, *args):
        gid = C.c_int()
        N.check(N.lib.lipasr_graph_begin(self.h.h, N.stream_ptr()))
        N.capture_enter()
        try:
            fn(*args)
        finally:
            try:
                N.check(N.lib.lipasr_graph_end(self.h.h, N.stream_ptr(), C.byref(gid)))
            finally:
                N.capture_exit()
        return gid.value

    def _warm_start(self):
        if self.constraint == "per_layer" and not self._warm:
            m = self.model
            N.check(N.lib.lipasr_mlp_project_per_layer(m._plan, N.ptr(m._params), self.rho, N.ptr(self.v_state), 0, 48, N.ptr(self.sigmas),
                                                       N.stream_ptr()))
            self._warm = True

    def profile_train(self, n_steps):
        self._prof = [(torch.cuda.Event(enable_timing=True), torch.cuda.Event(enable_timing=True)) for _ in range(int(n_steps))]
        self._prof_i = 0

    def train_ms(self):
        used = self._prof[:self._prof_i]
        self._prof = None
        if not used:
            return 0.0
        used[-1][1].synchronize()
        return sum(a.elapsed_time(b) for a, b in used) / len(used)

    def step(self, waves, y_onehot, features=None, global_batch=None):
        bsz = (features if features is not None else waves).shape[0]
        gb = int(global_batch) if global_batch is not None else bsz * self.dp.world
        b = self._i % self._nbuf
        self._i += 1
        self.feats, self.labels = self._feats2[b], self._labels2[b]
        if self._closed:
            raise RuntimeError("TrainPipeline.step() after close()")
        self._check_flags()
        caller = torch.cuda.current_stream(self.dev)
        xs = self.mfcc_stream
        idle = self.stream.query() if self._flags is not None else (self._last_train_ev is None or self._last_train_ev.query())
        wide = self._wide_stream is not None and features is None and idle
        if wide:
            xs = self._wide_stream
            self.ex.set(1, self._n_cu)
        if self.sync_inputs:
            xs.wait_stream(caller)
        with torch.cuda.stream(xs):
            if self._flags is not None:
                if self._last_xs is not None and self._last_xs is not xs:
                    xs.wait_stream(self._last_xs)
                self._last_xs = xs
            elif self._ev_last_mfcc is not None and self._wide_stream is not None:
                xs.wait_event(self._ev_last_mfcc)
            if self._flags is not None:
                fl = self._flags
                if self._i > self._nbuf:
                    N.check(N.lib.lipasr_flag_wait(self.h.h, fl[self._nbuf + b:].data_ptr(), self._i - self._nbuf, self._flag_timeout_ms, self._flag_err.data_ptr(), N.stream_ptr()))
            elif self._ev_free[b] is not None:
                xs.wait_event(self._ev_free[b])
            if features is not None:
                self._feats2[b][:bsz].copy_(features)
            else:
                if self._custom_ex:
                    self.ex(waves, self.mean, self.scale, out=self._feats2[b][:bsz])
                else:
                    self.ex(waves, self.L, self.mean, self.scale, out=self._feats2[b][:bsz])
            self._labels2[b][:bsz].copy_(y_onehot)
            if self._flags is not None:
                N.check(N.lib.lipasr_flag_signal(self.h.h, self._flags[b:].data_ptr(), self._i, N.stream_ptr()))
            else:
                self._ev_feat[b].record(xs)
                self._ev_last_mfcc = self._ev_feat[b]
        if wide:
            self.ex.set(1, self.mfcc_cus)
        if self.sync_inputs:
            if self._flags is not None:
                caller.wait_stream(xs)
            else:
                caller.wait_event(self._ev_feat[b])
        with torch.cuda.stream(self.stream):
            self._warm_start()
            if self._flags is not None:
                N.check(N.lib.lipasr_flag_wait(self.h.h, self._flags[b:].data_ptr(), self._i, self._flag_timeout_ms, self._flag_err.data_ptr(), N.stream_ptr()))
            else:
                self.stream.wait_event(self._ev_feat[b])
            prof = None
            if getattr(self, "_prof", None) is not None and self._prof_i < len(self._prof):
                prof = self._prof[self._prof_i]
                self._prof_i += 1
                prof[0].record(self.stream)
            if self.sync_bn:
                self._syncbn_step(bsz, b, gb)
            elif not self.use_graph:
                if self.dp.world == 1:
                    self._attack_and_train(bsz, b, gb)
                    self._update(self._flags[self._nbuf + b:].data_ptr() if self._adam_signal else None)
                elif self.overlap_buckets:
                    self._attack_and_train(bsz, b, gb, defer_dw0=True)
                    self._reduce_and_update_eager(bsz, b)
                else:
                    self._attack_and_train(bsz, b, gb)
                    self.dp.allreduce_grads(self.model._grads)
                    self._update()
            else:
                g = self._graphs.get((bsz, b, gb))
                if g is None:
                    if self.dp.world == 1:
                        g = (self._capture(lambda: (self._attack_and_train(bsz, b, gb), self._update())),)
                    elif self.overlap_buckets:
                        g = (self._capture(self._attack_and_train, bsz, b, gb, True), self._capture(self._dw0, bsz, b),
                             self._capture(self._update))
                    else:
                        g = (self._capture(self._attack_and_train, bsz, b, gb), self._capture(self._update))
                    self._graphs[(bsz, b, gb)] = g
                N.check(N.lib.lipasr_graph_launch(self.h.h, g[0], N.stream_ptr()))
                if len(g) == 3:
                    late = self._late
                    ha = self.dp.allreduce_async(self.model._grads[late:])
                    N.check(N.lib.lipasr_graph_launch(self.h.h, g[1], N.stream_ptr()))
                    hb = self.dp.allreduce_async(self.model._grads[:late])
                    ha.wait()
                    hb.wait()
                    N.check(N.lib.lipasr_graph_launch(self.h.h, g[2], N.stream_ptr()))
                elif len(g) == 2:
                    self.dp.allreduce_grads(self.model._grads)
                    N.check(N.lib.lipasr_graph_launch(self.h.h, g[1], N.stream_ptr()))
            if prof is not None:
                prof[1].record(self.stream)
            if self._adam_signal:
                pass
            elif self._flags is not None:
                N.check(N.lib.lipasr_flag_signal(self.h.h, self._flags[self._nbuf + b:].data_ptr(), self._i, N.stream_ptr()))
            else:
                ev = torch.cuda.Event()
                ev.record(self.stream)
                self._ev_free[b] = ev
                self._last_train_ev = ev

    def synchronize(self):
        if getattr(self, "_wide_stream", None) is not None:
            self._wide_stream.synchronize()
        self.mfcc_stream.synchronize()
        self.stream.synchronize()
        self._check_flags()
        if self.model.exchange_errors():
            raise RuntimeError("TrainPipeline: a BatchNorm exchange inside a GEMM gave up after 2 s (workgroups of one column block were never "
                               "resident together: is the plan's CU budget larger than its stream's CU mask?); the step's results are invalid. "
                               "LIPASR_FUSE_BN=0 uses the launch chain")

    @property
    def mfcc_stream_kind(self):
        return "masked" if self._masked_stream is not None else "shared"

    def close(self):
        if getattr(self, "_closed", True):
            return
        if N._capture_depth > 0:
            N._deferred.append((self.close, ()))
            return
        self._closed = True
        if not self.h.alive:
            self._graphs.clear()
            self._masked_stream = self._masked_train_stream = None
            self.stream = self.mfcc_stream = torch.cuda.current_stream(self.dev)
            return
        pending = None
        try:
            self.synchronize()
        except RuntimeError as e:
            pending = e
        for g in self._graphs.values():
            for gid in g:
                N.lib.lipasr_graph_destroy(self.h.h, gid)
        self._graphs.clear()
        st = self._masked_stream
        if st is not None:
            self._masked_stream = None
            self.mfcc_stream = torch.cuda.Stream(device=self.dev)
            N.lib.lipasr_stream_destroy(self.h.h, st)
        st = self._masked_train_stream
        if st is not None:
            self._masked_train_stream = None
            self.stream = torch.cuda.Stream(device=self.dev)
            N.lib.lipasr_stream_destroy(self.h.h, st)
        if self._gemm_tiles_set and getattr(self.model, "_plan", None):
            self._gemm_tiles_set = False
            N.lib.lipasr_mlp_set_gemm_tiles(self.model._plan, 0)
            N.lib.lipasr_mlp_set_cu_budget(self.model._plan, 0)
        if not self._custom_ex:
            self.ex.close()
        if pending is not None:
            raise pending

    def __del__(self):
        try:
            self.close()
        except Exception:
            pass
```

include/lipasr.h:

```cpp
#ifndef LIPASR_H
#define LIPASR_H

#include <stddef.h>
#include <stdint.h>

#ifdef __cplusplus
extern "C" {
#endif

#define LIPASR_OK            0
#define LIPASR_EINVAL       -1
#define LIPASR_ENOMEM       -2
#define LIPASR_EHIP         -3
#define LIPASR_EUNSUPPORTED -4
#define LIPASR_ESTATE       -5

#define LIPASR_MAX_LAYERS   16
#define LIPASR_N_MFCC       20
#define LIPASR_N_MELS       128
#define LIPASR_N_FFT        2048
#define LIPASR_HOP          512
#define LIPASR_SR           22050

typedef struct lipasr_ctx* lipasr_handle_t;
// ... 203 lines not shown
int lipasr_square_step(lipasr_handle_t h, const float* logits , const int* labels ,
                       const float* x0, const int* n_valid , int batch, int classes, int height, int width,
                       int win_h, int win_w, uint32_t p_q, int targeted, uint32_t clip0, uint32_t restart, uint32_t it, int flags,
                       uint64_t seed, float eps, float clip_lo, float clip_hi, float* x_best, float* x_cand,
                       float* loss_best , int* done , int* win , lipasr_stream_t stream);

int lipasr_square_init_host(const float* x0, const int* n_valid, int batch, int height, int width, uint32_t clip0, uint32_t restart,
                            uint64_t seed, float eps, float clip_lo, float clip_hi, float* x_best, float* x_cand, int* win);
int lipasr_square_step_host(const float* logits, const int* labels, const float* x0, const int* n_valid, int batch, int classes,
                            int height, int width, int win_h, int win_w, uint32_t p_q, int targeted, uint32_t clip0, uint32_t restart,
                            uint32_t it, int flags, uint64_t seed, float eps, float clip_lo, float clip_hi, float* x_best, float* x_cand,
                            float* loss_best, int* done, int* win);

int lipasr_hsj_expand(lipasr_handle_t h, const float* x , const float* delta ,
                      const int* n_valid , int batch, int n, int draws, uint32_t clip0, uint32_t it, uint32_t draw0,
                      uint64_t seed, float norm, float clip_lo, float clip_hi, float* out ,
                      lipasr_stream_t stream);

int lipasr_hsj_accumulate(lipasr_handle_t h, const float* logits, const int* labels , const float* p, const float* x,
                          const int* n_valid, int batch, int classes, int n, int draws, int targeted,
                          double* sums , int* counts , lipasr_stream_t stream);

int lipasr_hsj_direction(lipasr_handle_t h, const double* sums, const int* counts, const int* n_valid, int batch, int n, float norm,
                         float* u , lipasr_stream_t stream);

#define LIPASR_HSJ_START 0
#define LIPASR_HSJ_HALVE 1
#define LIPASR_HSJ_BISECT 2
#define LIPASR_HSJ_FIRST 1
#define LIPASR_HSJ_LAST 2
int lipasr_hsj_search(lipasr_handle_t h, const float* logits, const int* labels, const float* x0, const int* n_valid,
                      const float* u , const float* start_lo , const float* start_hi ,
                      const float* theta , int batch, int classes, int n, int mode, int flags, int targeted,
                      uint32_t clip0, uint32_t draw, uint64_t seed, float norm, float step_scale, int max_halvings, float clip_lo,
                      float clip_hi, float* x_cand, float* x_far, float* x_adv, float* x_best, float* fstate ,
                      int* istate , lipasr_stream_t stream);

int lipasr_hsj_expand_host(const float* x, const float* delta, const int* n_valid, int batch, int n, int draws, uint32_t clip0,
                           uint32_t it, uint32_t draw0, uint64_t seed, float norm, float clip_lo, float clip_hi, float* out);
int lipasr_hsj_accumulate_host(const float* logits, const int* labels, const float* p, const float* x, const int* n_valid, int batch,
                               int classes, int n, int draws, int targeted, double* sums, int* counts);
int lipasr_hsj_direction_host(const double* sums, const int* counts, const int* n_valid, int batch, int n, float norm, float* u);
int lipasr_hsj_search_host(const float* logits, const int* labels, const float* x0, const int* n_valid, const float* u,
                           const float* start_lo, const float* start_hi, const float* theta, int batch, int classes, int n, int mode,
                           int flags, int targeted, uint32_t clip0, uint32_t draw, uint64_t seed, float norm, float step_scale,
                           int max_halvings, float clip_lo, float clip_hi, float* x_cand, float* x_far, float* x_adv, float* x_best,
                           float* fstate, int* istate);
int lipasr_debug_hsj_path(int n, int aligned);

int lipasr_room_apply(const float* x, const int* n_valid, const float* rirs, int taps, int rir_count, int clips, int n, float* out,
                      lipasr_stream_t stream);
int lipasr_room_vjp(const float* g, const int* n_valid, const float* rirs, int taps, int rir_count, int clips, int n, float scale,
                    float* gx, lipasr_stream_t stream);
int lipasr_room_apply_host(const float* x, const int* n_valid, const float* rirs, int taps, int rir_count, int clips, int n,
                           float* out);
int lipasr_room_vjp_host(const float* g, const int* n_valid, const float* rirs, int taps, int rir_count, int clips, int n,
                         float scale, float* gx);

#define LIPASR_UNIVERSAL_GROUP 64

int lipasr_universal_shifts(lipasr_handle_t h, int batch, int P, uint32_t clip0, uint32_t it, uint64_t seed, int* offs_out ,
                            lipasr_stream_t stream);

int lipasr_universal_apply(lipasr_handle_t h, const float* x , const float* noise , const int* offs,
                           const int* n_valid, int batch, int n, int P, float clip_lo, float clip_hi, float* out ,
                           lipasr_stream_t stream);

int lipasr_universal_reduce(lipasr_handle_t h, const float* g , const int* offs, const int* n_valid, int batch, int n,
                            int P, double* sums , lipasr_stream_t stream);

int lipasr_universal_step(lipasr_handle_t h, float* noise , const double* sums , int groups, int P, float norm,
                          float alpha, float eps, lipasr_stream_t stream);

int lipasr_universal_shifts_host(int batch, int P, uint32_t clip0, uint32_t it, uint64_t seed, int* offs_out);
int lipasr_universal_apply_host(const float* x, const float* noise, const int* offs, const int* n_valid, int batch, int n, int P,
                                float clip_lo, float clip_hi, float* out);
int lipasr_universal_reduce_host(const float* g, const int* offs, const int* n_valid, int batch, int n, int P, double* sums);
int lipasr_universal_step_host(float* noise, const double* sums, int groups, int P, float norm, float alpha, float eps);

int lipasr_mlp_bounds_workspace(lipasr_mlp_t m, int batch, size_t* floats);
int lipasr_mlp_bounds(lipasr_mlp_t m, const float* params, const float* bnstate, const float* x ,
                      const float* eps , float norm, float clip_lo, float clip_hi, const int* y , int batch,
                      float* workspace, size_t workspace_floats, float* margin_ibp ,
                      float* margin_crown , float* slack , float* layer_lo ,
                      float* layer_hi , lipasr_stream_t stream);
int lipasr_mlp_bounds_workspace_host(int n_layers, const int* widths, int batch, size_t* floats);
int lipasr_mlp_bounds_host(int n_layers, const int* widths, const int* bn, const float* params, const float* bnstate, const float* x,
                           const float* eps, float norm, float clip_lo, float clip_hi, const int* y, int batch, float* workspace,
                           size_t workspace_floats, float* margin_ibp, float* margin_crown, float* slack, float* layer_lo,
                           float* layer_hi);
long lipasr_debug_bounds_launches(int kernel);

int lipasr_warp_apply(const float* x , const int* n_valid, const float* params ,
                      const float* table , int clips, int K, int n, float* out ,
                      lipasr_stream_t stream);
int lipasr_warp_param_vjp(const float* x, const float* g , const int* n_valid, const float* params,
                          const float* table, int clips, int K, int n, double* gp , lipasr_stream_t stream);
int lipasr_warp_table_host(float* win , float* delta );
int lipasr_warp_apply_host(const float* x, const int* n_valid, const float* params, const float* table, int clips, int K, int n,
                           float* out);
int lipasr_warp_param_vjp_host(const float* x, const float* g, const int* n_valid, const float* params, const float* table, int clips,
                               int K, int n, double* gp);
long lipasr_debug_warp_launches(int kernel);

#define LIPASR_DEFENCE_MEDIAN 0
#define LIPASR_DEFENCE_FIR 1
#define LIPASR_DEFENCE_QUANTIZE 2
#define LIPASR_DEFENCE_MAX_STAGES 4
#define LIPASR_DEFENCE_MAX_HALO 256
int lipasr_defence_apply(const float* x , const int* n_valid, const int* kinds ,
                         const int* args , const float* const* taps ,
                         int stages, int clips, int n, float* out , lipasr_stream_t stream);
int lipasr_defence_vjp(const float* x, const float* g , const int* n_valid, const int* kinds, const int* args,
                       const float* const* taps, int stages, int clips, int n, float* gx , lipasr_stream_t stream);
int lipasr_defence_apply_host(const float* x, const int* n_valid, const int* kinds, const int* args, const float* const* taps,
                              int stages, int clips, int n, float* out);
int lipasr_defence_vjp_host(const float* x, const float* g, const int* n_valid, const int* kinds, const int* args,
                            const float* const* taps, int stages, int clips, int n, float* gx);
long lipasr_debug_defence_launches(int kernel);

int lipasr_mlp_attack_step(lipasr_mlp_t m, const float* params, const float* bnstate, float* x_adv,
                           const float* x0, const float* y_onehot, int batch, float alpha, float eps,
                           lipasr_stream_t stream);

int lipasr_mlp_attack_step_lp(lipasr_mlp_t m, const float* params, const float* bnstate, float* x_adv, const float* x0,
                              const float* y_onehot, int batch, float norm, float alpha, float eps, lipasr_stream_t stream);

int lipasr_mlp_own_labels(lipasr_mlp_t m, const float* params, const float* bnstate, const float* x,
                          int batch, float* y_onehot_out, lipasr_stream_t stream);

int lipasr_mfcc_plan(lipasr_handle_t h, int sr_in, int n_samp, int batch_max);
int lipasr_mfcc_plan_ex(lipasr_handle_t h, int sr_in, int n_samp, int batch_max, int n_fft, int hop);
int lipasr_mfcc_dims(lipasr_handle_t h, int* n_y, int* n_frames);

int lipasr_mfcc_f32(lipasr_handle_t h, const float* wav, int batch, int utterance_length,
                    const double* affine_mean, const double* affine_scale, float* out,
                    lipasr_stream_t stream);
int lipasr_resample_f32(lipasr_handle_t h, const float* wav, int batch, float* y, lipasr_stream_t stream);
int lipasr_mfcc_from_22k(lipasr_handle_t h, const float* y, int batch, int n_y, int utterance_length,
                         const double* affine_mean, const double* affine_scale, float* out,
                         lipasr_stream_t stream);

int lipasr_mfcc_i16(lipasr_handle_t h, const int16_t* pcm, const int* n_valid, int batch,
                    int utterance_length, const double* affine_mean, const double* affine_scale,
                    float* out, lipasr_stream_t stream);

int lipasr_mfcc_create(lipasr_handle_t h, int sr_in, int n_samp_max, int batch_max, int n_fft, int hop,
                       lipasr_mfcc_t* out);
int lipasr_mfcc_destroy(lipasr_mfcc_t p);
int lipasr_mfcc_plan_dims(lipasr_mfcc_t p, int* n_y, int* n_frames, int* fused);
int lipasr_mfcc_extract(lipasr_mfcc_t p, const void* wav, int sample_format, const int* n_valid, int batch,
                        int utterance_length, const double* affine_mean, const double* affine_scale,
                        float* out, lipasr_stream_t stream);
int lipasr_mfcc_plan_resample(lipasr_mfcc_t p, const float* wav, int batch, float* y, lipasr_stream_t stream);
int lipasr_mfcc_plan_from_22k(lipasr_mfcc_t p, const float* y, int batch, int n_y, int utterance_length,
                              const double* affine_mean, const double* affine_scale, float* out,
                              lipasr_stream_t stream);

int lipasr_mfcc_plan_vjp(lipasr_mfcc_t p, const float* sig, int domain, int batch, int utterance_length,
                         const double* affine_scale, const float* g_feat, float* g_sig, int flags,
                         lipasr_stream_t stream);
int lipasr_mfcc_plan_vjp_ragged(lipasr_mfcc_t p, const void* sig, int sample_format, const int* n_valid, int domain,
                                int batch, int utterance_length, const double* affine_scale, const float* g_feat,
                                float* g_sig, int flags , lipasr_stream_t stream);
int lipasr_mfcc_plan_vjp_short(lipasr_mfcc_t p, const float* sig, int domain, int batch, int utterance_length,
                               const double* affine_scale, const float* g_feat, float* g_sig, int flags,
                               lipasr_stream_t stream);
int lipasr_mfcc_plan_resample_ragged(lipasr_mfcc_t p, const void* wav, int sample_format, const int* n_valid, int batch,
                                     float* y, lipasr_stream_t stream);
int lipasr_mfcc_plan_from_22k_ragged(lipasr_mfcc_t p, const float* y, const int* n_valid, int batch, int utterance_length,
                                     const double* affine_mean, const double* affine_scale, float* out,
                                     lipasr_stream_t stream);
int lipasr_mfcc_plan_resample_vjp(lipasr_mfcc_t p, const float* g_y, int batch, float* g_wav, lipasr_stream_t stream);

int lipasr_mfcc_profile_begin(lipasr_handle_t h, int max_calls);
int lipasr_mfcc_profile_end(lipasr_handle_t h, float* avg_ms3, int* n_calls);
int lipasr_mfcc_plan_profile_begin(lipasr_mfcc_t p, int max_calls);
int lipasr_mfcc_plan_profile_end(lipasr_mfcc_t p, float* avg_ms3, int* n_calls);
int lipasr_mfcc_plan_set(lipasr_mfcc_t p, int key, int value);

int lipasr_dolphin_create(lipasr_handle_t h, int sr_in, int n_samp_max, int batch_max, double carrier_hz, double carrier_level,
                          lipasr_dolphin_t* out);
int lipasr_dolphin_destroy(lipasr_dolphin_t p);
int lipasr_dolphin_bandpass(lipasr_dolphin_t p, const float* wav, const int* n_valid, int batch, float* voice, lipasr_stream_t stream);
int lipasr_dolphin_generate(lipasr_dolphin_t p, const float* wav, const int* n_valid, int batch, float* ultrasound, float* peaks_or_null,
                            lipasr_stream_t stream);
int lipasr_dolphin_record(lipasr_dolphin_t p, const float* ultrasound, const int* n_valid, int batch, float a1, float a2, float* rec,
                          lipasr_stream_t stream);
int lipasr_dolphin_generate_recorded(lipasr_dolphin_t p, const float* wav, const int* n_valid, int batch, float a1, float a2,
                                     float* rec, lipasr_stream_t stream);
int lipasr_dolphin_table(int which, int sr_in, double* out, int cap);

int lipasr_psy_create(lipasr_handle_t h, int sample_rate, int n_max, int batch_max, int flags ,
                      lipasr_psy_t* out);
int lipasr_psy_destroy(lipasr_psy_t p);
int lipasr_psy_psd(lipasr_psy_t p, const float* x, int n, int batch, float* psd, float* psd_max, lipasr_stream_t stream);
int lipasr_psy_threshold(lipasr_psy_t p, const float* psd, int n_frames, int batch, float* theta, int* n_maskers_or_null,
                         lipasr_stream_t stream);
int lipasr_psy_prepare(lipasr_psy_t p, const float* x, int n, int batch, float* theta, float* psd_max, lipasr_stream_t stream);
int lipasr_psy_loss_grad(lipasr_psy_t p, const float* delta, int n, int batch, const float* theta, const float* psd_max, float* loss,
                         float* g_delta_or_null, lipasr_stream_t stream);
int lipasr_psy_step(lipasr_psy_t p, float* delta, float* x_adv, const float* x0, const float* g_net, const float* g_theta_or_null,
                    const float* alpha_or_null, const float* eps, int n, int batch, float lr, int use_sign, float clip_lo, float clip_hi,
                    lipasr_stream_t stream);
int lipasr_psy_table(int which, int sample_rate, double* out, int cap);

int lipasr_add_noise_f32(lipasr_handle_t h, float* y, int batch, int n, int mode, float p0, float p1,
                         uint64_t seed, lipasr_stream_t stream);

int lipasr_debug_set(lipasr_handle_t h, int key, int value);

int lipasr_debug_gemm_mode(int mode);

long lipasr_debug_launch_count(int kind);

long lipasr_debug_gemm_launches(int kind, int exchange, int amode, int bmode, int arith, int epi);

long lipasr_debug_group_launches(int family, int arith, int variant);

int lipasr_debug_gemm(lipasr_handle_t h, int arith, int transA, int transB, int M, int N, int K, const float* A, int lda,
                      const float* B, int ldb, float* C, int ldc, float scale_a, float scale_b, lipasr_stream_t stream);

long lipasr_debug_k3_launches(int kernel);

long lipasr_debug_k1_launches(int kernel);

int lipasr_debug_mfcc_stage(lipasr_mfcc_t p, int which, int batch, float* out, lipasr_stream_t stream);

long lipasr_debug_k1_vjp_launches(int kernel);

int lipasr_debug_mfcc_vjp_stage(lipasr_mfcc_t p, int which, int batch, float* out, lipasr_stream_t stream);

int lipasr_debug_mfcc_stage_put(lipasr_mfcc_t p, int which, int batch, const float* in, lipasr_stream_t stream);

long lipasr_debug_k2_launches(int kernel);

int lipasr_debug_mlp_stage(lipasr_mlp_t m, int layer, int which, int batch, float* out, lipasr_stream_t stream);

int lipasr_debug_chain_head(int n);

int lipasr_debug_table(int which, int sr_in, float* out, int cap);

#ifdef __cplusplus
}
#endif
#endif
```

Measured before the change: 3.237 million utterances/sec.

## Add half-LDS DCT kernel and fold label copy into DCT launch

After: 3.234 million utterances/sec, median of 2. Within noise of the previous version (-0.1%).

```diff
diff --git a/asr-using-robust-nn_amd/csrc/core.hip b/asr-using-robust-nn_amd/csrc/core.hip
--- a/asr-using-robust-nn_amd/csrc/core.hip
+++ b/asr-using-robust-nn_amd/csrc/core.hip
@@ -48,7 +48,7 @@
 
 extern "C" {
 
-int lipasr_version(void) { return 740; }
+int lipasr_version(void) { return 750; }
 
 const char* lipasr_last_error(void) { return g_err; }
 
diff --git a/asr-using-robust-nn_amd/csrc/mfcc.hip b/asr-using-robust-nn_amd/csrc/mfcc.hip
--- a/asr-using-robust-nn_amd/csrc/mfcc.hip
+++ b/asr-using-robust-nn_amd/csrc/mfcc.hip
@@ -247,12 +247,16 @@
 }
 
 static int plan_run(MfccPlan* p, const void* wav, int fmt, const int* n_valid, int batch, int L, const double* am, const double* as,
-                    float* out, hipStream_t st) {
+                    float* out, hipStream_t st, DctRider rider = DctRider()) {
   LP_CHECK_ARG(wav && out, "lipasr_mfcc: null argument");
   LP_CHECK_ARG(fmt == 0 || fmt == 1, "lipasr_mfcc: sample format %d (0 = float32, 1 = int16 PCM)", fmt);
   LP_CHECK_ARG((am == nullptr) == (as == nullptr), "lipasr_mfcc: give both affine arrays or neither");
   const MfccPath path = pick_mfcc_path(p, wav, fmt, n_valid != nullptr);
   if (path.rc != LIPASR_OK) return path.rc;
+  if (rider.src && !path.fused && from_22k_fuses_dct(p, path.stft, L)) {
+    set_error("lipasr_mfcc_extract_rider: the plan ends with the block-DFT kernel's own DCT epilogue (plan key 4), which carries no rider");
+    return LIPASR_EUNSUPPORTED;
+  }
   hipEvent_t* ev = p->prof_half ? nullptr : prof_slot(p);
   int rc;
   if (ev) LP_HIP(hipEventRecord(ev[EV_RESAMPLE_BEGIN], st));
@@ -263,14 +267,15 @@
     }
     if ((rc = launch_fused(p, wav, fmt, n_valid, batch, st)) != LIPASR_OK) return rc;
     if (ev) LP_HIP(hipEventRecord(ev[EV_STFT_END], st));
-    if ((rc = launch_dct(p, batch, L, am, as, out, n_valid, st)) != LIPASR_OK) return rc;
+    if ((rc = launch_dct(p, batch, L, am, as, out, n_valid, st, rider)) != LIPASR_OK) return rc;
   } else {
     if ((rc = launch_resample(p, path.resampler, wav, fmt, n_valid, batch, p->d_y, st)) != LIPASR_OK) return rc;
     if (ev) {
       LP_HIP(hipEventRecord(ev[EV_RESAMPLE_END], st));
       LP_HIP(hipEventRecord(ev[EV_STFT_BEGIN], st));
     }
-    if ((rc = launch_from_22k(p, path.stft, p->d_y, n_valid, batch, L, am, as, out, st, ev ? ev[EV_STFT_END] : nullptr)) != LIPASR_OK) return rc;
+    if ((rc = launch_from_22k(p, path.stft, p->d_y, n_valid, batch, L, am, as, out, st, ev ? ev[EV_STFT_END] : nullptr, false, rider)) != LIPASR_OK)
+      return rc;
   }
   if (ev) {
     LP_HIP(hipEventRecord(ev[EV_DCT_END], st));
@@ -606,6 +611,21 @@
   return plan_run(p, wav, sample_format, n_valid, batch, utterance_length, affine_mean, affine_scale, out, S(stream));
 }
 
+int lipasr_mfcc_extract_rider(lipasr_mfcc_t p, const void* wav, int sample_format, const int* n_valid, int batch, int utterance_length,
+                              const double* affine_mean, const double* affine_scale, float* out, const float* rider_src, float* rider_dst,
+                              int rider_rows, int rider_cols, lipasr_stream_t stream) {
+  int rc = plan_check("lipasr_mfcc_extract_rider", p, batch, utterance_length);
+  if (rc != LIPASR_OK) return rc;
+  LP_CHECK_ARG((rider_src == nullptr) == (rider_dst == nullptr), "lipasr_mfcc_extract_rider: give both rider arrays or neither");
+  DctRider rider;
+  if (rider_src) {
+    LP_CHECK_ARG(rider_rows == batch, "lipasr_mfcc_extract_rider: %d rider rows for a batch of %d (one row per clip)", rider_rows, batch);
+    LP_CHECK_ARG(rider_cols >= 0, "lipasr_mfcc_extract_rider: rider_cols=%d", rider_cols);
+    rider.src = rider_src; rider.dst = rider_dst; rider.cols = rider_cols;
+  }
+  return plan_run(p, wav, sample_format, n_valid, batch, utterance_length, affine_mean, affine_scale, out, S(stream), rider);
+}
+
 int lipasr_mfcc_plan_resample(lipasr_mfcc_t p, const float* wav, int batch, float* y, lipasr_stream_t stream) {
   int rc = plan_check("lipasr_mfcc_plan_resample", p, batch, 1);
   if (rc != LIPASR_OK) return rc;
@@ -677,6 +697,13 @@
   DeviceGuard g(p->ctx->device);
   LP_HIP(hipMemcpyAsync(out, src, (size_t)batch * row * sizeof(float), hipMemcpyDeviceToDevice, S(stream)));
   return LIPASR_OK;
+}
+
+int lipasr_debug_dct_residency(lipasr_mfcc_t p, int utterance_length, int affine, int* wg_size, int* lds_bytes, int* wgs_per_cu) {
+  LP_CHECK_ARG(p != nullptr && wg_size && lds_bytes && wgs_per_cu, "lipasr_debug_dct_residency: null argument");
+  LP_CHECK_ARG(utterance_length >= 1, "lipasr_debug_dct_residency: utterance_length=%d", utterance_length);
+  DeviceGuard g(p->ctx->device);
+  return dct_residency(utterance_length, affine != 0, wg_size, lds_bytes, wgs_per_cu);
 }
 
 long lipasr_debug_k1_vjp_launches(int kernel) { return (kernel >= 0 && kernel < K1V_KERNELS) ? g_k1_vjp_launches[kernel] : -1; }
diff --git a/asr-using-robust-nn_amd/csrc/mfcc_plan.h b/asr-using-robust-nn_amd/csrc/mfcc_plan.h
--- a/asr-using-robust-nn_amd/csrc/mfcc_plan.h
+++ b/asr-using-robust-nn_amd/csrc/mfcc_plan.h
@@ -117,11 +117,20 @@
 int launch_resample(const MfccPlan* p, MfccPath::Resampler kind, const void* wav, int fmt, const int* n_valid, int batch, float* y,
                     hipStream_t st);
 int launch_clear_tail(const MfccPlan* p, const int* n_valid, int batch, float* y, hipStream_t st);
+struct DctRider {
+  const float* src = nullptr;
+  float* dst = nullptr;
+  int cols = 0;
+};
 std::vector<float> dct_fragments();
 void fill_stft_args(const MfccPlan* p, const float* y, StftArgs* a);
-int launch_dct(const MfccPlan* p, int batch, int L, const double* am, const double* as, float* out, const int* n_valid, hipStream_t st);
+int launch_dct(const MfccPlan* p, int batch, int L, const double* am, const double* as, float* out, const int* n_valid, hipStream_t st,
+               DctRider rider = DctRider());
+int dct_residency(int L, bool affine, int* wg_size, int* lds_bytes, int* wgs_per_cu);
+bool from_22k_fuses_dct(const MfccPlan* p, MfccPath::Stft kind, int L);
 int launch_from_22k(const MfccPlan* p, MfccPath::Stft kind, const float* y, const int* n_valid, int batch, int L, const double* am,
-                    const double* as, float* out, hipStream_t st, hipEvent_t mid = nullptr, bool stft_only = false);
+                    const double* as, float* out, hipStream_t st, hipEvent_t mid = nullptr, bool stft_only = false,
+                    DctRider rider = DctRider());
 int launch_mfcc_vjp_db(const MfccVjpArgs& a, hipStream_t st);
 struct ShortVjpArgs {
   const float* y;
diff --git a/asr-using-robust-nn_amd/csrc/stft_mel.hip b/asr-using-robust-nn_amd/csrc/stft_mel.hip
--- a/asr-using-robust-nn_amd/csrc/stft_mel.hip
+++ b/asr-using-robust-nn_amd/csrc/stft_mel.hip
@@ -495,28 +495,95 @@
 
 
 constexpr int kDctFrames = 64;
-
-__global__ __launch_bounds__(128) void dct_kernel(const float* __restrict__ db, const float* __restrict__ frame_max,
-                                                   int n_frames, int L, int chunk, const float4* __restrict__ dct_frag,
-                                                   const double* __restrict__ aff_mean,
-                                                   const double* __restrict__ aff_scale, float* __restrict__ out,
-                                                   const int* __restrict__ n_valid, int n_samp_max, int sr_in) {
+constexpr int kDctHalfFrames = 48;
+
+struct DctArgs {
+  const float* db;
+  const float* frame_max;
+  int n_frames, L, chunk;
+  const float4* dct_frag;
+  const double* aff_mean;
+  const double* aff_scale;
+  float* out;
+  const int* n_valid;
+  int n_samp_max, sr_in;
+  DctRider rider;
+};
+
+__device__ __forceinline__ int dct_clip_frames(const DctArgs& a, int u) {
+  int nf = a.n_frames;
+  if (a.n_valid) {
+    int nvy, ny;
+    clip_lengths(min(max(a.n_valid[u], 0), a.n_samp_max), a.sr_in, &nvy, &ny, &nf);
+    nf = min(nf, a.n_frames);
+  }
+  return nf;
+}
+
+__device__ __forceinline__ void dct_rider_copy(const DctRider& r, int u, int tid) {
+  if (r.src == nullptr || blockIdx.y != 0) return;
+  const size_t o = (size_t)u * r.cols;
+  for (int c = tid; c < r.cols; c += 128) r.dst[o + c] = r.src[o + c];
+}
+
+__device__ __forceinline__ float dct_frame_max0(const DctArgs& a, int u, int nf, int tid) {
+  return tid < nf ? a.frame_max[(size_t)u * a.n_frames + tid] : -INFINITY;
+}
+__device__ __forceinline__ float dct_floor(const DctArgs& a, int u, int nf, int tid, float fm0, float* red) {
+  float mx = fmaxf(-INFINITY, fm0);
+  for (int t = tid + 128; t < nf; t += 128) mx = fmaxf(mx, a.frame_max[(size_t)u * a.n_frames + t]);
+  mx = wave_max(mx);
+  if ((tid & 63) == 0) red[tid >> 6] = mx;
+  __syncthreads();
+  return fmaxf(red[0], red[1]) - 80.0f;
+}
+
+constexpr int kDctRowsPerLane = 12;
+struct DctAffine { double mean[kDctRowsPerLane], scale[kDctRowsPerLane]; };
+__device__ __forceinline__ void dct_affine_load(const DctArgs& a, int t0, int tl, int tid, DctAffine* f) {
+  const int li = tid & 31, h = (tid >> 5) & 1, t = (tid >> 6) * 32 + li;
+#pragma unroll
+  for (int q = 0; q < kDctRowsPerLane; ++q) {
+    const int c = (q & 3) + 8 * (q >> 2) + 4 * h;
+    const int oo = (t < tl && c < kNMfcc) ? c * a.L + t0 + t : 0;
+    f->mean[q] = a.aff_mean[oo];
+    f->scale[q] = a.aff_scale[oo];
+  }
+}
+
+template <bool kAffineLoaded>
+__device__ __forceinline__ void dct_store(const DctArgs& a, const rs_f32x16& acc, int u, int t0, int tl, int tu, int tid, const DctAffine* f) {
+  const int li = tid & 31, h = (tid >> 5) & 1, t = (tid >> 6) * 32 + li;
+  const int n_out = kNMfcc * a.L;
+  if (t < tl) {
+#pragma unroll
+    for (int q = 0; q < kDctRowsPerLane; ++q) {
+      const int c = (q & 3) + 8 * (q >> 2) + 4 * h;
+      if (c < kNMfcc) {
+        float v = (t < tu) ? acc[q] : 0.0f;
+        const int oo = c * a.L + t0 + t;
+        if (kAffineLoaded) v = (float)(((double)v - f->mean[q]) / f->scale[q]);
+        else if (a.aff_mean) v = (float)(((double)v - a.aff_mean[oo]) / a.aff_scale[oo]);
+        a.out[(size_t)u * n_out + oo] = v;
+      }
+    }
+  }
+}
+
+__global__ __launch_bounds__(128) void dct_kernel(const DctArgs a) {
   extern __shared__ float dbs[];
   __shared__ float red[2];
   const int tid = threadIdx.x, lane = tid & 63, wave = tid >> 6, u = blockIdx.x;
   const int li = lane & 31, h = lane >> 5;
+  const int chunk = a.chunk;
   const int t0 = blockIdx.y * chunk;
-  const int tl = min(chunk, L - t0);
-  int nf = n_frames;
-  if (n_valid) {
-    int nvy, ny;
-    clip_lengths(min(max(n_valid[u], 0), n_samp_max), sr_in, &nvy, &ny, &nf);
-    nf = min(nf, n_frames);
-  }
+  const int tl = min(chunk, a.L - t0);
+  const int nf = dct_clip_frames(a, u);
   const int tu = max(0, min(nf - t0, tl));
   const int tp = chunk + 1;
-  const float* src = db + ((size_t)u * n_frames + t0) * 128;
+  const float* src = a.db + ((size_t)u * a.n_frames + t0) * 128;
   const int n_live = tu * 128;
+  const float fm0 = dct_frame_max0(a, u, nf, tid);
   float stage[kDctFrames];
 #pragma unroll
   for (int j = 0; j < kDctFrames; ++j) {
@@ -524,15 +591,11 @@
     stage[j] = (i < n_live) ? src[i] : 0.0f;
   }
   float4 av4[16];
-  const float4* ap = dct_frag + (li * 2 + h) * 16;
+  const float4* ap = a.dct_frag + (li * 2 + h) * 16;
 #pragma unroll
   for (int s4 = 0; s4 < 16; ++s4) av4[s4] = ap[s4];
-  float mx = -INFINITY;
-  for (int t = tid; t < nf; t += 128) mx = fmaxf(mx, frame_max[(size_t)u * n_frames + t]);
-  mx = wave_max(mx);
-  if (lane == 0) red[wave] = mx;
-  __syncthreads();
-  const float thr = fmaxf(red[0], red[1]) - 80.0f;
+  dct_rider_copy(a.rider, u, tid);
+  const float thr = dct_floor(a, u, nf, tid, fm0, red);
 #pragma unroll
   for (int j = 0; j < kDctFrames; ++j) {
     const int i = tid + 128 * j;
@@ -549,20 +612,69 @@
 #pragma unroll
     for (int e = 0; e < 4; ++e) acc = __builtin_amdgcn_mfma_f32_32x32x2f32(a4[e], bp[2 * (4 * s4 + e) * tp], acc, 0, 0, 0);
   }
-  const int t = wave * 32 + li;
-  const int n_out = kNMfcc * L;
-  if (t < tl) {
-#pragma unroll
-    for (int q = 0; q < 16; ++q) {
-      const int c = (q & 3) + 8 * (q >> 2) + 4 * h;
-      if (c < kNMfcc) {
-        float v = (t < tu) ? acc[q] : 0.0f;
-        const int oo = c * L + t0 + t;
-        if (aff_mean) v = (float)(((double)v - aff_mean[oo]) / aff_scale[oo]);
-        out[(size_t)u * n_out + oo] = v;
-      }
-    }
-  }
+  dct_store<false>(a, acc, u, t0, tl, tu, tid, nullptr);
+}
+
+constexpr int kDctHalfStride = kDctHalfFrames + 1;
+constexpr size_t kDctHalfLds = (size_t)64 * kDctHalfStride * sizeof(float);
+
+template <bool kAffine>
+__global__ __launch_bounds__(128, 4) void dct_half_kernel(const DctArgs a) {
+  extern __shared__ float dbs[];
+  __shared__ float red[2];
+  const int tid = threadIdx.x, lane = tid & 63, u = blockIdx.x;
+  const int wave = __builtin_amdgcn_readfirstlane(tid >> 6);
+  const int li = lane & 31, h = lane >> 5;
+  const int chunk = a.chunk;
+  const int t0 = blockIdx.y * chunk;
+  const int tl = min(chunk, a.L - t0);
+  const int nf = dct_clip_frames(a, u);
+  const int tu = max(0, min(nf - t0, tl));
+  constexpr int tp = kDctHalfStride;
+  const float fm0 = dct_frame_max0(a, u, nf, tid);
+  const float* src = a.db + ((size_t)u * a.n_frames + t0) * 128 + lane;
+  float stage[2][kDctHalfFrames / 2];
+#pragma unroll
+  for (int jj = 0; jj < kDctHalfFrames / 2; ++jj) {
+    const int f = 2 * jj + wave;
+    stage[0][jj] = (f < tu) ? src[f * 128] : 0.0f;
+    stage[1][jj] = (f < tu) ? src[f * 128 + 64] : 0.0f;
+  }
+  float4 av4[8], aw4[8];
+  const float4* ap = a.dct_frag + (li * 2 + h) * 16;
+#pragma unroll
+  for (int s4 = 0; s4 < 8; ++s4) av4[s4] = ap[s4];
+  dct_rider_copy(a.rider, u, tid);
+  const float thr = dct_floor(a, u, nf, tid, fm0, red);
+  rs_f32x16 acc;
+#pragma unroll
+  for (int q = 0; q < 16; ++q) acc[q] = 0.0f;
+  float* wp = dbs + lane * tp + wave;
+  const float* bp = dbs + h * tp + min(wave * 32 + li, chunk - 1);
+#pragma unroll
+  for (int jj = 0; jj < kDctHalfFrames / 2; ++jj) wp[2 * jj] = (2 * jj + wave < tu) ? fmaxf(stage[0][jj], thr) : 0.0f;
+  __syncthreads();
+#pragma unroll
+  for (int s4 = 0; s4 < 8; ++s4) aw4[s4] = ap[8 + s4];
+#pragma unroll
+  for (int s4 = 0; s4 < 8; ++s4) {
+    const float a4[4] = {av4[s4].x, av4[s4].y, av4[s4].z, av4[s4].w};
+#pragma unroll
+    for (int e = 0; e < 4; ++e) acc = __builtin_amdgcn_mfma_f32_32x32x2f32(a4[e], bp[2 * (4 * s4 + e) * tp], acc, 0, 0, 0);
+  }
+  __syncthreads();
+#pragma unroll
+  for (int jj = 0; jj < kDctHalfFrames / 2; ++jj) wp[2 * jj] = (2 * jj + wave < tu) ? fmaxf(stage[1][jj], thr) : 0.0f;
+  __syncthreads();
+  DctAffine aff;
+  if (kAffine) dct_affine_load(a, t0, tl, tid, &aff);
+#pragma unroll
+  for (int s4 = 0; s4 < 8; ++s4) {
+    const float a4[4] = {aw4[s4].x, aw4[s4].y, aw4[s4].z, aw4[s4].w};
+#pragma unroll
+    for (int e = 0; e < 4; ++e) acc = __builtin_amdgcn_mfma_f32_32x32x2f32(a4[e], bp[2 * (4 * s4 + e) * tp], acc, 0, 0, 0);
+  }
+  dct_store<kAffine>(a, acc, u, t0, tl, tu, tid, &aff);
 }
 
 std::vector<float> dct_fragments() {
@@ -574,14 +686,38 @@
   return f;
 }
 
+struct DctPick { int chunk; size_t lds; bool half; };
+static DctPick pick_dct(int L) {
+  DctPick k;
+  k.chunk = std::min(kDctFrames, (L + 3) & ~3);
+  k.half = k.chunk <= kDctHalfFrames;
+  k.lds = k.half ? kDctHalfLds : (size_t)128 * (k.chunk + 1) * sizeof(float);
+  return k;
+}
+
 int launch_dct(const MfccPlan* p, int batch, int L, const double* am, const double* as, float* out, const int* n_valid,
-                      hipStream_t st) {
-  const int chunk = std::min(kDctFrames, (L + 3) & ~3);
-  const size_t lds = (size_t)128 * (chunk + 1) * sizeof(float);
-  hipLaunchKernelGGL(dct_kernel, dim3(batch, (L + chunk - 1) / chunk), dim3(128), lds, st, p->d_db, p->d_fmax, p->n_frames, L, chunk,
-                     reinterpret_cast<const float4*>(p->d_dct), am, as, out, n_valid, p->n_samp, p->sr_in);
+                      hipStream_t st, DctRider rider) {
+  const DctPick k = pick_dct(L);
+  DctArgs a;
+  a.db = p->d_db; a.frame_max = p->d_fmax; a.n_frames = p->n_frames; a.L = L; a.chunk = k.chunk;
+  a.dct_frag = reinterpret_cast<const float4*>(p->d_dct); a.aff_mean = am; a.aff_scale = as; a.out = out; a.n_valid = n_valid;
+  a.n_samp_max = p->n_samp; a.sr_in = p->sr_in; a.rider = rider;
+  const dim3 grid(batch, (L + k.chunk - 1) / k.chunk);
+  if (!k.half) hipLaunchKernelGGL(dct_kernel, grid, dim3(128), k.lds, st, a);
+  else if (am) hipLaunchKernelGGL(dct_half_kernel<true>, grid, dim3(128), k.lds, st, a);
+  else hipLaunchKernelGGL(dct_half_kernel<false>, grid, dim3(128), k.lds, st, a);
   ++g_k1_launches[K1_DCT];
   LP_LAUNCH_CHECK();
+  return LIPASR_OK;
+}
+
+int dct_residency(int L, bool affine, int* wg_size, int* lds_bytes, int* wgs_per_cu) {
+  const DctPick k = pick_dct(L);
+  int n = 0;
+  if (!k.half) LP_HIP(hipOccupancyMaxActiveBlocksPerMultiprocessor(&n, dct_kernel, 128, k.lds));
+  else if (affine) LP_HIP(hipOccupancyMaxActiveBlocksPerMultiprocessor(&n, dct_half_kernel<true>, 128, k.lds));
+  else LP_HIP(hipOccupancyMaxActiveBlocksPerMultiprocessor(&n, dct_half_kernel<false>, 128, k.lds));
+  *wg_size = 128; *lds_bytes = (int)k.lds; *wgs_per_cu = n;
   return LIPASR_OK;
 }
 
@@ -594,8 +730,12 @@
   a->n_valid = nullptr; a->sr_in = p->sr_in; a->n_samp_max = p->n_samp;
 }
 
+bool from_22k_fuses_dct(const MfccPlan* p, MfccPath::Stft kind, int L) {
+  return kind == MfccPath::ST_BDFT && p->bd_fuse_dct && bdft_can_fuse_dct(p->n_frames, p->bd_seg, L);
+}
+
 int launch_from_22k(const MfccPlan* p, MfccPath::Stft kind, const float* y, const int* n_valid, int batch, int L, const double* am,
-                    const double* as, float* out, hipStream_t st, hipEvent_t mid, bool stft_only) {
+                    const double* as, float* out, hipStream_t st, hipEvent_t mid, bool stft_only, DctRider rider) {
   StftArgs a;
   fill_stft_args(p, y, &a);
   a.n_valid = n_valid;
@@ -614,7 +754,7 @@
       break;
     }
     case MfccPath::ST_BDFT: {
-      const bool fuse = !stft_only && p->bd_fuse_dct && bdft_can_fuse_dct(p->n_frames, p->bd_seg, L);
+      const bool fuse = !stft_only && from_22k_fuses_dct(p, kind, L);
       BdftDct d;
       d.L = L; d.dct_frag = reinterpret_cast<const float4*>(p->d_dct); d.aff_mean = am; d.aff_scale = as; d.out = out;
       const int rc = launch_stft_bdft(a, p->bd, batch, p->bd_seg, fuse ? &d : nullptr, st);
@@ -637,7 +777,7 @@
   LP_LAUNCH_CHECK();
   if (mid) LP_HIP(hipEventRecord(mid, st));
   if (stft_only) return LIPASR_OK;
-  return launch_dct(p, batch, L, am, as, out, n_valid, st);
-}
-
-}
+  return launch_dct(p, batch, L, am, as, out, n_valid, st, rider);
+}
+
+}
diff --git a/asr-using-robust-nn_amd/lipasr/_native.py b/asr-using-robust-nn_amd/lipasr/_native.py
--- a/asr-using-robust-nn_amd/lipasr/_native.py
+++ b/asr-using-robust-nn_amd/lipasr/_native.py
@@ -162,6 +162,7 @@
     "lipasr_mfcc_destroy": (i32, [c_h]),
     "lipasr_mfcc_plan_dims": (i32, [c_h, PI, PI, PI]),
     "lipasr_mfcc_extract": (i32, [c_h, c_f, i32, c_f, i32, i32, c_f, c_f, c_f, c_s]),
+    "lipasr_mfcc_extract_rider": (i32, [c_h, c_f, i32, c_f, i32, i32, c_f, c_f, c_f, c_f, c_f, i32, i32, c_s]),
     "lipasr_mfcc_plan_resample": (i32, [c_h, c_f, i32, c_f, c_s]),
     "lipasr_mfcc_plan_from_22k": (i32, [c_h, c_f, i32, i32, i32, c_f, c_f, c_f, c_s]),
     "lipasr_mfcc_plan_vjp": (i32, [c_h, c_f, i32, i32, i32, c_f, c_f, c_f, i32, c_s]),
@@ -199,6 +200,7 @@
     "lipasr_debug_k3_launches": (C.c_long, [i32]),
     "lipasr_debug_k1_launches": (C.c_long, [i32]),
     "lipasr_debug_mfcc_stage": (i32, [c_h, i32, i32, c_f, c_s]),
+    "lipasr_debug_dct_residency": (i32, [c_h, i32, i32, PI, PI, PI]),
     "lipasr_debug_k1_vjp_launches": (C.c_long, [i32]),
     "lipasr_debug_mfcc_vjp_stage": (i32, [c_h, i32, i32, c_f, c_s]),
     "lipasr_debug_mfcc_stage_put": (i32, [c_h, i32, i32, c_f, c_s]),
@@ -232,7 +234,8 @@
          "lipasr_mlp_bounds_workspace_host": 710, "lipasr_mlp_bounds_host": 710, "lipasr_debug_bounds_launches": 710, "lipasr_warp_table_host": 720,
          "lipasr_warp_apply": 720, "lipasr_warp_param_vjp": 720, "lipasr_warp_apply_host": 720, "lipasr_warp_param_vjp_host": 720,
          "lipasr_debug_warp_launches": 720, "lipasr_debug_k2_launches": 730, "lipasr_debug_mlp_stage": 730, "lipasr_defence_apply": 740,
-         "lipasr_defence_vjp": 740, "lipasr_defence_apply_host": 740, "lipasr_defence_vjp_host": 740, "lipasr_debug_defence_launches": 740}
+         "lipasr_defence_vjp": 740, "lipasr_defence_apply_host": 740, "lipasr_defence_vjp_host": 740, "lipasr_debug_defence_launches": 740,
+         "lipasr_mfcc_extract_rider": 750, "lipasr_debug_dct_residency": 750}
 lib.lipasr_version.restype = i32
 _VERSION = lib.lipasr_version()
 
diff --git a/asr-using-robust-nn_amd/lipasr/extract_features_construct_dataset.py b/asr-using-robust-nn_amd/lipasr/extract_features_construct_dataset.py
--- a/asr-using-robust-nn_amd/lipasr/extract_features_construct_dataset.py
+++ b/asr-using-robust-nn_amd/lipasr/extract_features_construct_dataset.py
@@ -29,6 +29,7 @@
         ny, nf, fu = C.c_int(), C.c_int(), C.c_int()
         N.check(N.lib.lipasr_mfcc_plan_dims(plan, C.byref(ny), C.byref(nf), C.byref(fu)))
         self.n_y, self.n_frames, self.fused = ny.value, nf.value, bool(fu.value)
+        self.fuse_dct = False
 
     def close(self):
         plan, self._plan = getattr(self, "_plan", None), None
@@ -41,8 +42,16 @@
         except Exception:
             pass
 
+    def dct_residency(self, utterance_length=STANDARD_UTTERANCE_LENGTH, affine=False):
+        wg, lds, per_cu = C.c_int(), C.c_int(), C.c_int()
+        N.check(N.lib.lipasr_debug_dct_residency(self._plan, int(utterance_length), 1 if affine else 0, C.byref(wg), C.byref(lds),
+                                                 C.byref(per_cu)))
+        return wg.value, lds.value, per_cu.value
+
     def set(self, key, value):
         N.check(N.lib.lipasr_mfcc_plan_set(self._plan, int(key), int(value)))
+        if int(key) == 4:
+            self.fuse_dct = bool(value)
 
     def profile_begin(self, max_calls):
         N.check(N.lib.lipasr_mfcc_plan_profile_begin(self._plan, int(max_calls)))
@@ -52,7 +61,7 @@
         N.check(N.lib.lipasr_mfcc_plan_profile_end(self._plan, ms3, C.byref(n)))
         return {"resample": ms3[0], "stft_mel": ms3[1], "dct": ms3[2]}, n.value
 
-    def __call__(self, waves, utterance_length=STANDARD_UTTERANCE_LENGTH, mean=None, scale=None, out=None, n_valid=None):
+    def __call__(self, waves, utterance_length=STANDARD_UTTERANCE_LENGTH, mean=None, scale=None, out=None, n_valid=None, rider=None):
         if self._plan is None:
             raise RuntimeError("MfccExtractor used after close()")
         b = waves.shape[0]
@@ -68,6 +77,14 @@
             raise ValueError("n_valid must be an int32 device tensor [B]")
         if out is None:
             out = torch.empty(b, N_MFCC * utterance_length, device=self.device)
+        if rider is not None:
+            src, dst = rider
+            if (src.dim() != 2 or dst.dim() != 2 or src.shape[0] != b or dst.shape[0] < b or dst.shape[1] != src.shape[1]
+                    or src.dtype != torch.float32 or dst.dtype != torch.float32 or not src.is_contiguous() or not dst.is_contiguous()):
+                raise ValueError(f"rider must be contiguous float32 (src [{b}, cols], dst [>= {b}, cols])")
+            N.check(N.lib.lipasr_mfcc_extract_rider(self._plan, N.ptr(waves), fmt, N.ptr(n_valid), b, utterance_length, N.ptr(mean),
+                                                    N.ptr(scale), N.ptr(out), N.ptr(src), N.ptr(dst), b, src.shape[1], N.stream_ptr()))
+            return out
         N.check(N.lib.lipasr_mfcc_extract(self._plan, N.ptr(waves), fmt, N.ptr(n_valid), b, utterance_length, N.ptr(mean), N.ptr(scale),
                                           N.ptr(out), N.stream_ptr()))
         return out
diff --git a/asr-using-robust-nn_amd/lipasr/pipeline.py b/asr-using-robust-nn_amd/lipasr/pipeline.py
--- a/asr-using-robust-nn_amd/lipasr/pipeline.py
+++ b/asr-using-robust-nn_amd/lipasr/pipeline.py
@@ -75,6 +75,8 @@
         self._adam_signal = (self._flags is not None and self.dp.world == 1 and not self.sync_bn and not self.use_graph
                              and self.constraint == "product" and N.has("lipasr_mlp_adam_project_product_signal")
                              and _os.environ.get("LIPASR_ADAM_SIGNAL", "1") == "1")
+        self._label_rider = (not self._custom_ex and N.has("lipasr_mfcc_extract_rider")
+                             and _os.environ.get("LIPASR_LABEL_RIDER", "1") == "1")
         self._ev_feat = [torch.cuda.Event() for _ in range(self._nbuf)]
         self._ev_free = [None] * self._nbuf
         self._i = 0
@@ -328,14 +330,19 @@
                     N.check(N.lib.lipasr_flag_wait(self.h.h, fl[self._nbuf + b:].data_ptr(), self._i - self._nbuf, self._flag_timeout_ms, self._flag_err.data_ptr(), N.stream_ptr()))
             elif self._ev_free[b] is not None:
                 xs.wait_event(self._ev_free[b])
+            ride = (self._label_rider and features is None and not self.ex.fuse_dct and torch.is_tensor(y_onehot)
+                    and y_onehot.dtype == torch.float32 and y_onehot.is_cuda and y_onehot.is_contiguous()
+                    and tuple(y_onehot.shape) == (bsz, self._labels2[b].shape[1]))
             if features is not None:
                 self._feats2[b][:bsz].copy_(features)
             else:
                 if self._custom_ex:
                     self.ex(waves, self.mean, self.scale, out=self._feats2[b][:bsz])
                 else:
-                    self.ex(waves, self.L, self.mean, self.scale, out=self._feats2[b][:bsz])
-            self._labels2[b][:bsz].copy_(y_onehot)
+                    self.ex(waves, self.L, self.mean, self.scale, out=self._feats2[b][:bsz],
+                            rider=(y_onehot, self._labels2[b]) if ride else None)
+            if not ride:
+                self._labels2[b][:bsz].copy_(y_onehot)
             if self._flags is not None:
                 N.check(N.lib.lipasr_flag_signal(self.h.h, self._flags[b:].data_ptr(), self._i, N.stream_ptr()))
             else:
diff --git a/include/lipasr.h b/include/lipasr.h
--- a/include/lipasr.h
+++ b/include/lipasr.h
@@ -379,6 +379,9 @@
 int lipasr_mfcc_extract(lipasr_mfcc_t p, const void* wav, int sample_format, const int* n_valid, int batch,
                         int utterance_length, const double* affine_mean, const double* affine_scale,
                         float* out, lipasr_stream_t stream);
+int lipasr_mfcc_extract_rider(lipasr_mfcc_t p, const void* wav, int sample_format, const int* n_valid, int batch,
+                              int utterance_length, const double* affine_mean, const double* affine_scale, float* out,
+                              const float* rider_src, float* rider_dst, int rider_rows, int rider_cols, lipasr_stream_t stream);
 int lipasr_mfcc_plan_resample(lipasr_mfcc_t p, const float* wav, int batch, float* y, lipasr_stream_t stream);
 int lipasr_mfcc_plan_from_22k(lipasr_mfcc_t p, const float* y, int batch, int n_y, int utterance_length,
                               const double* affine_mean, const double* affine_scale, float* out,
@@ -454,6 +457,8 @@
 
 int lipasr_debug_mfcc_stage(lipasr_mfcc_t p, int which, int batch, float* out, lipasr_stream_t stream);
 
+int lipasr_debug_dct_residency(lipasr_mfcc_t p, int utterance_length, int affine, int* wg_size, int* lds_bytes, int* wgs_per_cu);
+
 long lipasr_debug_k1_vjp_launches(int kernel);
 
 int lipasr_debug_mfcc_vjp_stage(lipasr_mfcc_t p, int which, int batch, float* out, lipasr_stream_t stream);
```
